# facebookresearch/theseus

Measured on NVIDIA H100. Metric: LM iterations/sec on batched SE3 pose-graph (2500 poses, global batch 2048 over N GPUs, LM + block-sparse Cholesky, fp64), higher is better.
Workload: dtype f64

## Files before the change

### include/thb200.h

```cpp
#ifndef THB200_H_
#define THB200_H_

#include <stdint.h>

#ifdef __cplusplus
extern "C" {
#endif

typedef struct CUstream_st* thb_stream_t;

#define THB_OK 0
#define THB_ERR_BAD_ARG (-1)
#define THB_ERR_UNSUPPORTED (-2)
#define THB_ERR_ALLOC (-3)

int thb_version(void);
int thb_compiled_arch(void);
int64_t thb_launch_count(void);

enum thb_cost_kind {
  THB_COST_BETWEEN_SE3 = 0,
  THB_COST_LOCAL_SE3 = 1,
  THB_COST_BETWEEN_SO3 = 2,
  THB_COST_LOCAL_SO3 = 3,
  THB_COST_LOCAL_VECTOR = 4,
  THB_COST_BETWEEN_SE2 = 6,
  THB_COST_LOCAL_SE2 = 7,
  THB_COST_REPROJECTION = 5
};
enum thb_robust_kind { THB_ROBUST_NONE = 0, THB_ROBUST_WELSCH = 1, THB_ROBUST_HUBER = 2 };
enum thb_weight_kind {
  THB_WEIGHT_SCALE = 0,
  THB_WEIGHT_DIAGONAL = 1
};
enum thb_var_kind { THB_VAR_SE3 = 0, THB_VAR_SO3 = 1, THB_VAR_VECTOR = 2, THB_VAR_SE2 = 3, THB_VAR_SO2 = 4 };

typedef struct thb_cost_group {
  int32_t kind;
  int32_t weight_kind;
  int32_t K;
  int32_t dim;
  const void* const* x0;
  const void* const* x1;
  const void* const* aux;
  const void* const* w;
  const int32_t* bstride;
  const int64_t* a_off;
  const int32_t* a_stride;
  const int32_t* bp;
  const int32_t* row0;
  const void* const* aux2;
  const void* const* aux3;
  const void* const* aux4;
  const int32_t* bstride2;
  int32_t robust_kind;
  int32_t reserved0;
  const void* const* log_radius;
  const int32_t* bstride_lr;
} thb_cost_group;

int thb_linearize_group_f64(const thb_cost_group* g, int64_t B, double* A_val, int64_t nnz, double* b, int64_t m,
                            thb_stream_t stream);
int thb_linearize_group_f32(const thb_cost_group* g, int64_t B, float* A_val, int64_t nnz, float* b, int64_t m,
                            thb_stream_t stream);

int thb_error_num_chunks(int32_t K);
int thb_error_group_f64(const thb_cost_group* g, int64_t B, double* partial, thb_stream_t stream);
int thb_error_group_f32(const thb_cost_group* g, int64_t B, float* partial, thb_stream_t stream);
int thb_error_reduce_f64(const double* partial, int32_t num_chunks, int64_t B, double* err, thb_stream_t stream);
int thb_error_reduce_f32(const float* partial, int32_t num_chunks, int64_t B, float* err, thb_stream_t stream);

typedef struct thb_var_table {
  int32_t N;
  const void* const* x;
  void* const* out;
  const int32_t* kind;
  const int32_t* col;
  const int32_t* dof;
} thb_var_table;

int thb_retract_f64(const thb_var_table* vt, int64_t B, const double* delta, int64_t n, double step,
                    const uint8_t* ignore , thb_stream_t stream);
int thb_retract_f32(const thb_var_table* vt, int64_t B, const float* delta, int64_t n, float step,
                    const uint8_t* ignore, thb_stream_t stream);
int thb_commit_f64(const thb_var_table* vt, int64_t B, const uint8_t* keep_old, thb_stream_t stream);
int thb_commit_f32(const thb_var_table* vt, int64_t B, const uint8_t* keep_old, thb_stream_t stream);

typedef struct thb_gram_plan {
  int64_t num_entries;
  const int32_t* ent_blk;
  const int16_t* ent_p;
  const int16_t* ent_q;
  const int64_t* blk_out;
  const int32_t* blk_ld;
  const int64_t* blk_mirror;
  const int32_t* blk_cptr;
  const int64_t* c_off;
  const int32_t* c_stride;
  const int32_t* c_rows;
  const int32_t* c_bpa;
  const int32_t* c_bpb;
  int64_t n;
  const int32_t* col_cptr;
  const int64_t* cc_off;
  const int32_t* cc_stride;
  const int32_t* cc_rows;
  const int32_t* cc_row0;
  int64_t num_blocks;
  const int32_t* blk_rows;
  const int32_t* blk_cols;
  int64_t num_segments;
  const int32_t* segments;
  const int32_t* blk_order;
} thb_gram_plan;

int thb_gram_f64(const thb_gram_plan* p, int64_t B, const double* A_val, int64_t nnz, const double* b, int64_t m,
                 double* out, int64_t out_bstride, double* Atb, double* diag, thb_stream_t stream);
int thb_gram_f32(const thb_gram_plan* p, int64_t B, const float* A_val, int64_t nnz, const float* b, int64_t m,
                 float* out, int64_t out_bstride, float* Atb, float* diag, thb_stream_t stream);
int thb_fill_zero(void* ptr, int64_t bytes, thb_stream_t stream);

int64_t thb_potrf_workspace_bytes(int64_t B, int64_t n);
int thb_potrf_f64(const double* AtA, const double* alpha, const double* beta, int32_t* info, int64_t B, int64_t n,
                  void* workspace, int64_t workspace_bytes, thb_stream_t stream);
int thb_potrs_f64(const double* rhs, double* x, int64_t B, int64_t n, const void* workspace, int64_t workspace_bytes,
                  thb_stream_t stream);
int thb_potrf_potrs_f64(const double* AtA, const double* rhs, const double* alpha, const double* beta, double* x,
                        int32_t* info, int64_t B, int64_t n, void* workspace, int64_t workspace_bytes,
                        thb_stream_t stream);

typedef struct thb_sparse_plan {
  int32_t N;
  int32_t num_levels;
  int32_t max_dim;
  int32_t reserved;
  int64_t n;
  int64_t data_size;
  int64_t winv_size;
  const int32_t* dims;
  const int32_t* col_start;
  const int32_t* pstart;
  const int64_t* winv_off;
  const int64_t* diag_off;
  const int64_t* up_a;
  const int64_t* up_b;
  const int32_t* up_k;
  const int64_t* u_ptr;
  const int64_t* u_tgt; const int16_t* u_r; const int16_t* u_c; const int16_t* u_ld; const int64_t* u_p0; const int64_t* u_p1;
  const int64_t* f_ptr;
  const int64_t* f_off; const int32_t* f_dim; const int64_t* f_w; const int32_t* f_col;
  const int64_t* t_ptr;
  const int64_t* t_off; const int16_t* t_r; const int16_t* t_dim; const int64_t* t_w;
  const int64_t* s_ptr;
  const int32_t* s_col;
  const int64_t* fr_ptr; const int64_t* fr_off; const int32_t* fr_k;
  const int64_t* bc_ptr; const int64_t* bc_off; const int32_t* bc_i;
} thb_sparse_plan;

int thb_sparse_damp_f64(const thb_sparse_plan* p, double* factor, const double* alpha, const double* beta, int64_t B,
                        thb_stream_t stream);
int thb_sparse_factor_f64(const thb_sparse_plan* p, double* factor, double* winv, int32_t* info, int64_t B, thb_stream_t stream);
int thb_sparse_solve_f64(const thb_sparse_plan* p, const double* factor, const double* winv, const double* rhs, double* x,
                         double* work, int64_t B, thb_stream_t stream);

typedef struct thb_symbolic thb_symbolic;
int thb_symbolic_create(const int64_t* param_size, int64_t N, const int64_t* blk_ptrs, const int64_t* blk_inds, int32_t ordering,
                        thb_symbolic** out);
void thb_symbolic_destroy(thb_symbolic* s);
int64_t thb_symbolic_array_count(const thb_symbolic* s, const char* name);
int32_t thb_symbolic_array_elem_bytes(const thb_symbolic* s, const char* name);
int thb_symbolic_array_copy(const thb_symbolic* s, const char* name, void* dst, int64_t dst_bytes);
double thb_symbolic_stat(const thb_symbolic* s, const char* name);

enum { THB_LANE_U = 0, THB_LANE_T = 1, THB_LANE_S = 2, THB_LANE_UH = 3, THB_LANE_TU = 4  };
typedef struct thb_sparse_lane_plan {
  int64_t N;
  int64_t n;
  int64_t data_size;
  int64_t diag_size;
  int64_t num_launches;
  const int32_t* launches;
  const int32_t* dims;
  const int32_t* col_start;
  const int32_t* pstart;
  const int64_t* dl_off;
  const int64_t* diag_off;
  const int64_t* up_a; const int64_t* up_b; const int32_t* up_k;
  const int64_t* u_tgt; const int64_t* u_p0; const int64_t* u_p1;
  const int64_t* t_off; const int64_t* t_diag; const int64_t* t_dl;
  const int32_t* t_pstart;
  const int32_t* s_col;
  const int64_t* fr_ptr; const int64_t* fr_off; const int32_t* fr_p; const int32_t* fr_d;
  const int64_t* bc_ptr; const int64_t* bc_off; const int32_t* bc_p; const int32_t* bc_d;
} thb_sparse_lane_plan;

int64_t thb_sparse_lane_padded_batch(int64_t B);
int thb_sparse_lane_gram_f64(const thb_gram_plan* g, int64_t B, const double* A_val, int64_t nnz, double* factor, thb_stream_t stream);
int thb_sparse_lane_damp_f64(const thb_sparse_lane_plan* p, double* factor, const double* alpha, const double* beta, int64_t B,
                             thb_stream_t stream);
int thb_sparse_lane_factor_f64(const thb_sparse_lane_plan* p, double* factor, double* diagl, int32_t* info, int64_t B,
                               thb_stream_t stream);
typedef struct thb_sparse_lane_root {
  int64_t num_blocks;
  int64_t num_cols;
  int64_t nt;
  int64_t root_start;
  int64_t num_segments;
  const int32_t* segments;
  const int64_t* rb_off; const int32_t* rb_row; const int32_t* rb_col; const int32_t* rb_di; const int32_t* rb_dj;
  const int64_t* rf_p0; const int64_t* rf_p1;
  const int32_t* root_cols;
  const int32_t* root_dims;
} thb_sparse_lane_root;
int thb_sparse_lane_root_gather_f64(const thb_sparse_lane_root* r, const double* factor, double* S, int64_t B, thb_stream_t stream);
int thb_sparse_lane_forward_f64(const thb_sparse_lane_plan* p, const double* factor, const double* diagl, const double* rhs, double* work,
                                int64_t B, thb_stream_t stream);
int thb_sparse_lane_backward_f64(const thb_sparse_lane_plan* p, const double* factor, const double* diagl, double* work, double* x, int64_t B,
                                 thb_stream_t stream);
int thb_sparse_lane_root_rhs_f64(const thb_sparse_lane_plan* p, const thb_sparse_lane_root* r, const double* factor, const double* rhs,
                                 const double* work, double* rhs_dense, int64_t B, thb_stream_t stream);
int thb_sparse_lane_root_scatter_f64(const thb_sparse_lane_plan* p, const thb_sparse_lane_root* r, const double* x_dense, double* work, double* x,
                                     int64_t B, thb_stream_t stream);
#define THB_TILE_ROWS 4
#define THB_TILE_COLS 4
typedef struct thb_sparse_lane_tiles {
  int64_t num_tiles, num_steps;
  const int64_t* tile_tgt;
  const int64_t* step_ptr;
  const int64_t* step_src;
} thb_sparse_lane_tiles;
int thb_sparse_lane_factor_tiled_f64(const thb_sparse_lane_plan* p, const thb_sparse_lane_tiles* t, double* factor, double* diagl,
                                     int32_t* info, int64_t B, thb_stream_t stream);
typedef struct thb_sparse_lane_pieces {
  int64_t num_pieces, num_launches;
  const int32_t* launches;
  const int64_t* first;
  const int32_t* width;
  const int64_t* fr_ext_end;
  const int64_t* bc_int_end;
  const int64_t* order;
} thb_sparse_lane_pieces;
int thb_sparse_lane_piece_forward_f64(const thb_sparse_lane_plan* p, const thb_sparse_lane_pieces* pc, const double* factor, const double* diagl,
                                      const double* rhs, double* work, int64_t B, thb_stream_t stream);
int thb_sparse_lane_piece_backward_f64(const thb_sparse_lane_plan* p, const thb_sparse_lane_pieces* pc, const double* factor, const double* diagl,
                                       double* work, double* x, int64_t B, thb_stream_t stream);
int thb_sparse_lane_solve_f64(const thb_sparse_lane_plan* p, const double* factor, const double* diagl, const double* rhs,
                              double* x, double* work, int64_t B, thb_stream_t stream);

int thb_lm_control_f64(const double* delta, const double* Atb, const double* diag, int64_t B, int64_t n, double step,
                       const double* err_prev, const double* err_new, double* lam, int32_t ellipsoidal,
                       double damping_accept, double down_ratio, double up_ratio, uint8_t* reject,
                       double* err_out, int32_t* stats, thb_stream_t stream);

int thb_lm_control_f32(const float* delta, const float* Atb, const float* diag, int64_t B, int64_t n, float step,
                       const float* err_prev, const float* err_new, float* lam, int32_t ellipsoidal, float damping_accept,
                       float down_ratio, float up_ratio, uint8_t* reject, float* err_out, int32_t* stats, thb_stream_t stream);

int thb_gram_dense_f64(const double* A, double* AtA, int64_t B, int64_t m, int64_t n, thb_stream_t stream);

typedef struct thb_front_plan {
  int64_t S;
  int64_t n;
  int64_t data_size;
  int64_t arena_size;
  int64_t varena_size;
  const int32_t* f_w; const int32_t* f_b; const int32_t* f_first; const int32_t* f_class;
  const int32_t* f_wpad; const int32_t* f_np; const int32_t* f_cb_ld; const int32_t* f_depth;
  const int64_t* f_panel_off; const int64_t* f_cb_off; const int64_t* f_fr_off; const int64_t* f_u_off;
  const int32_t* child_ptr; const int32_t* child_list;
  const int64_t* rel_ptr; const int32_t* f_rel;
  const int64_t* rows_ptr; const int32_t* f_rows;
  const int32_t* sched;
  const int32_t* perm;
  const int32_t* c_jw; const int64_t* c_sp_ptr; const int32_t* c_sp;
  const int64_t* c_inv_ptr; const int32_t* c_inv;
  const int64_t* fd; const int64_t* pc;
  const int32_t* pmap;
} thb_front_plan;

#define THB_FRONT_LAUNCH_COLS 12
int64_t thb_front_small_smem_bytes(int32_t w, int32_t b, int32_t nchildren);
int thb_front_factor_f64(const thb_front_plan* p, const int64_t* launches, int64_t num_launches, double* factor, const double* ata,
                         int64_t ata_stride, const double* alpha, const double* beta, double* arena, void* dense_ws, int64_t dense_ws_bytes,
                         int32_t* info, int64_t B, thb_stream_t stream);
int thb_front_solve_f64(const thb_front_plan* p, const int64_t* launches, int64_t num_launches, const double* factor, const double* rhs,
                        double* x, double* work, double* varena, int64_t B, thb_stream_t stream);
int64_t thb_potrf_partial_workspace_bytes(int64_t B, int64_t np);
int thb_potrf_partial_inplace_f64(double* F, int64_t bstride, int64_t np, int32_t nb_piv, int32_t w_real, int32_t n_real, int32_t info_base,
                                  int32_t* info, int64_t B, void* workspace, int64_t workspace_bytes, thb_stream_t stream);

int thb_mat_vec_f64(int64_t B, int64_t num_rows, int64_t num_cols, const int64_t* row_ptr, const int64_t* col_ind,
                    const double* A_val, const double* v, double* y, thb_stream_t stream);
int thb_tmat_vec_f64(int64_t B, int64_t num_rows, int64_t num_cols, const int64_t* row_ptr, const int64_t* col_ind,
                     const double* A_val, const double* v, double* y, thb_stream_t stream);

int thb_solve_backward_f64(int64_t B, int64_t num_rows, int64_t num_cols, const int64_t* row_ptr, const int64_t* col_ind,
                           const double* A_val, const double* b, const double* x, const double* H, const double* alpha,
                           int32_t detach_hessian, double* A_grad, double* b_grad, thb_stream_t stream);

int thb_se3_exp_f64(const double* tangent, double* group, int64_t N, thb_stream_t stream);
int thb_se3_log_f64(const double* group, double* tangent, double* jlog , int64_t N, thb_stream_t stream);
int thb_se3_adjoint_f64(const double* group, double* adj, int64_t N, thb_stream_t stream);
int thb_se3_inverse_f64(const double* group, double* out, int64_t N, thb_stream_t stream);
int thb_se3_compose_f64(const double* g0, const double* g1, double* out, int64_t N, thb_stream_t stream);
int thb_se3_exp_f32(const float* tangent, float* group, int64_t N, thb_stream_t stream);
int thb_se3_log_f32(const float* group, float* tangent, float* jlog, int64_t N, thb_stream_t stream);
int thb_se3_adjoint_f32(const float* group, float* adj, int64_t N, thb_stream_t stream);
int thb_se3_inverse_f32(const float* group, float* out, int64_t N, thb_stream_t stream);
int thb_se3_compose_f32(const float* g0, const float* g1, float* out, int64_t N, thb_stream_t stream);

int thb_so3_exp_f64(const double* tangent, double* group, int64_t N, thb_stream_t stream);
int thb_so3_log_f64(const double* group, double* tangent, double* jlog , int64_t N, thb_stream_t stream);
int thb_so3_adjoint_f64(const double* group, double* adj, int64_t N, thb_stream_t stream);
int thb_so3_inverse_f64(const double* group, double* out, int64_t N, thb_stream_t stream);
int thb_so3_compose_f64(const double* g0, const double* g1, double* out, int64_t N, thb_stream_t stream);
int thb_se2_exp_f64(const double* tangent, double* group, int64_t N, thb_stream_t stream);
int thb_se2_log_f64(const double* group, double* tangent, double* jlog , int64_t N, thb_stream_t stream);
int thb_se2_adjoint_f64(const double* group, double* adj, int64_t N, thb_stream_t stream);
int thb_se2_inverse_f64(const double* group, double* out, int64_t N, thb_stream_t stream);
int thb_se2_compose_f64(const double* g0, const double* g1, double* out, int64_t N, thb_stream_t stream);
int thb_so3_exp_f32(const float* tangent, float* group, int64_t N, thb_stream_t stream);
int thb_so3_log_f32(const float* group, float* tangent, float* jlog , int64_t N, thb_stream_t stream);
int thb_so3_adjoint_f32(const float* group, float* adj, int64_t N, thb_stream_t stream);
int thb_so3_inverse_f32(const float* group, float* out, int64_t N, thb_stream_t stream);
int thb_so3_compose_f32(const float* g0, const float* g1, float* out, int64_t N, thb_stream_t stream);
int thb_se2_exp_f32(const float* tangent, float* group, int64_t N, thb_stream_t stream);
int thb_se2_log_f32(const float* group, float* tangent, float* jlog , int64_t N, thb_stream_t stream);
int thb_se2_adjoint_f32(const float* group, float* adj, int64_t N, thb_stream_t stream);
int thb_se2_inverse_f32(const float* group, float* out, int64_t N, thb_stream_t stream);
int thb_se2_compose_f32(const float* g0, const float* g1, float* out, int64_t N, thb_stream_t stream);

int thb_so3_jexp_f64(const double* tangent, double* group , double* jexp, int64_t N, thb_stream_t stream);
int thb_se3_jexp_f64(const double* tangent, double* group , double* jexp, int64_t N, thb_stream_t stream);
int thb_so3_jexp_f32(const float* tangent, float* group , float* jexp, int64_t N, thb_stream_t stream);
int thb_se3_jexp_f32(const float* tangent, float* group , float* jexp, int64_t N, thb_stream_t stream);

#ifdef __cplusplus
}
#endif
#endif
```

### theseus_b200/_lib.py

```python
import ctypes as C
import os

_HERE = os.path.dirname(os.path.abspath(__file__))
_LIB_PATH = os.environ.get("THB200_LIB") or os.path.join(_HERE, "lib", "libthb200.so")
_lib = None

c_i32, c_i64, c_f64, c_f32, c_vp = C.c_int32, C.c_int64, C.c_double, C.c_float, C.c_void_p


class CostGroup(C.Structure):
    _fields_ = [("kind", c_i32), ("weight_kind", c_i32), ("K", c_i32), ("dim", c_i32),
                ("x0", c_vp), ("x1", c_vp), ("aux", c_vp), ("w", c_vp), ("bstride", c_vp),
                ("a_off", c_vp), ("a_stride", c_vp), ("bp", c_vp), ("row0", c_vp),
                ("aux2", c_vp), ("aux3", c_vp), ("aux4", c_vp), ("bstride2", c_vp),
                ("robust_kind", c_i32), ("reserved0", c_i32), ("log_radius", c_vp), ("bstride_lr", c_vp)]


class VarTable(C.Structure):
    _fields_ = [("N", c_i32), ("x", c_vp), ("out", c_vp), ("kind", c_vp), ("col", c_vp), ("dof", c_vp)]


class GramPlan(C.Structure):
    _fields_ = [("num_entries", c_i64), ("ent_blk", c_vp), ("ent_p", c_vp), ("ent_q", c_vp),
                ("blk_out", c_vp), ("blk_ld", c_vp), ("blk_mirror", c_vp), ("blk_cptr", c_vp),
                ("c_off", c_vp), ("c_stride", c_vp), ("c_rows", c_vp), ("c_bpa", c_vp), ("c_bpb", c_vp),
                ("n", c_i64), ("col_cptr", c_vp), ("cc_off", c_vp), ("cc_stride", c_vp), ("cc_rows", c_vp),
                ("cc_row0", c_vp), ("num_blocks", c_i64), ("blk_rows", c_vp), ("blk_cols", c_vp),
                ("num_segments", c_i64), ("segments", c_vp), ("blk_order", c_vp)]


def make_gram_plan(arrs, dev):
    return GramPlan(
        num_entries=int(arrs["ent_blk"].shape[0]), ent_blk=dev["ent_blk"].data_ptr(), ent_p=dev["ent_p"].data_ptr(),
        ent_q=dev["ent_q"].data_ptr(), blk_out=dev["blk_out"].data_ptr(), blk_ld=dev["blk_ld"].data_ptr(),
        blk_mirror=dev["blk_mirror"].data_ptr(), blk_cptr=dev["blk_cptr"].data_ptr(), c_off=dev["c_off"].data_ptr(),
        c_stride=dev["c_stride"].data_ptr(), c_rows=dev["c_rows"].data_ptr(), c_bpa=dev["c_bpa"].data_ptr(),
        c_bpb=dev["c_bpb"].data_ptr(), n=int(arrs["n"]), col_cptr=dev["col_cptr"].data_ptr(),
        cc_off=dev["cc_off"].data_ptr(), cc_stride=dev["cc_stride"].data_ptr(), cc_rows=dev["cc_rows"].data_ptr(),
        cc_row0=dev["cc_row0"].data_ptr(), num_blocks=int(arrs["blk_out"].shape[0]), blk_rows=dev["blk_rows"].data_ptr(),
        blk_cols=dev["blk_cols"].data_ptr(), num_segments=int(arrs["segments"].shape[0]), segments=arrs["segments"].ctypes.data,
        blk_order=dev["blk_order"].data_ptr())


class SparsePlanStruct(C.Structure):
    _fields_ = [("N", c_i32), ("num_levels", c_i32), ("max_dim", c_i32), ("reserved", c_i32),
                ("n", c_i64), ("data_size", c_i64), ("winv_size", c_i64)] + [(k, c_vp) for k in (
                    "dims", "col_start", "pstart", "winv_off", "diag_off", "up_a", "up_b", "up_k",
                    "u_ptr", "u_tgt", "u_r", "u_c", "u_ld", "u_p0", "u_p1",
                    "f_ptr", "f_off", "f_dim", "f_w", "f_col",
                    "t_ptr", "t_off", "t_r", "t_dim", "t_w",
                    "s_ptr", "s_col", "fr_ptr", "fr_off", "fr_k", "bc_ptr", "bc_off", "bc_i")]


class SparseLanePlanStruct(C.Structure):
    _fields_ = [("N", c_i64), ("n", c_i64), ("data_size", c_i64), ("diag_size", c_i64), ("num_launches", c_i64)] + [(k, c_vp) for k in (
        "launches", "dims", "col_start", "pstart", "dl_off", "diag_off", "up_a", "up_b", "up_k", "u_tgt", "u_p0", "u_p1",
        "t_off", "t_diag", "t_dl", "t_pstart", "s_col", "fr_ptr", "fr_off", "fr_p", "fr_d", "bc_ptr", "bc_off", "bc_p", "bc_d")]


_PG, _PV, _PP = C.POINTER(CostGroup), C.POINTER(VarTable), C.POINTER(GramPlan)
_PS = C.POINTER(SparsePlanStruct)
_PL = C.POINTER(SparseLanePlanStruct)


class SparseLaneRootStruct(C.Structure):
    _fields_ = [("num_blocks", c_i64), ("num_cols", c_i64), ("nt", c_i64), ("root_start", c_i64), ("num_segments", c_i64)] + [(k, c_vp) for k in (
        "segments", "rb_off", "rb_row", "rb_col", "rb_di", "rb_dj", "rf_p0", "rf_p1", "root_cols", "root_dims")]


class SparseLaneTilesStruct(C.Structure):
    _fields_ = [("num_tiles", c_i64), ("num_steps", c_i64), ("tile_tgt", c_vp), ("step_ptr", c_vp), ("step_src", c_vp)]


class SparseLanePiecesStruct(C.Structure):
    _fields_ = [("num_pieces", c_i64), ("num_launches", c_i64)] + [(k, c_vp) for k in (
        "launches", "first", "width", "fr_ext_end", "bc_int_end", "order")]


class FrontPlanStruct(C.Structure):
    _fields_ = [("S", c_i64), ("n", c_i64), ("data_size", c_i64), ("arena_size", c_i64), ("varena_size", c_i64)] + [(k, c_vp) for k in (
        "f_w", "f_b", "f_first", "f_class", "f_wpad", "f_np", "f_cb_ld", "f_depth", "f_panel_off", "f_cb_off", "f_fr_off", "f_u_off",
        "child_ptr", "child_list", "rel_ptr", "f_rel", "rows_ptr", "f_rows", "sched", "perm", "c_jw", "c_sp_ptr", "c_sp", "c_inv_ptr", "c_inv", "fd", "pc", "pmap")]


_PF = C.POINTER(FrontPlanStruct)
_PR = C.POINTER(SparseLaneRootStruct)
_PPIECES = C.POINTER(SparseLanePiecesStruct)
_PT = C.POINTER(SparseLaneTilesStruct)
SIGNATURES = {
    "thb_version": (c_i32, []),
    "thb_compiled_arch": (c_i32, []),
    "thb_launch_count": (c_i64, []),
    "thb_linearize_group_f64": (c_i32, [_PG, c_i64, c_vp, c_i64, c_vp, c_i64, c_vp]),
    "thb_linearize_group_f32": (c_i32, [_PG, c_i64, c_vp, c_i64, c_vp, c_i64, c_vp]),
    "thb_error_num_chunks": (c_i32, [c_i32]),
    "thb_error_group_f64": (c_i32, [_PG, c_i64, c_vp, c_vp]),
    "thb_error_group_f32": (c_i32, [_PG, c_i64, c_vp, c_vp]),
    "thb_error_reduce_f64": (c_i32, [c_vp, c_i32, c_i64, c_vp, c_vp]),
    "thb_error_reduce_f32": (c_i32, [c_vp, c_i32, c_i64, c_vp, c_vp]),
    "thb_retract_f64": (c_i32, [_PV, c_i64, c_vp, c_i64, c_f64, c_vp, c_vp]),
    "thb_retract_f32": (c_i32, [_PV, c_i64, c_vp, c_i64, c_f32, c_vp, c_vp]),
    "thb_commit_f64": (c_i32, [_PV, c_i64, c_vp, c_vp]),
    "thb_commit_f32": (c_i32, [_PV, c_i64, c_vp, c_vp]),
    "thb_gram_f64": (c_i32, [_PP, c_i64, c_vp, c_i64, c_vp, c_i64, c_vp, c_i64, c_vp, c_vp, c_vp]),
    "thb_gram_f32": (c_i32, [_PP, c_i64, c_vp, c_i64, c_vp, c_i64, c_vp, c_i64, c_vp, c_vp, c_vp]),
    "thb_fill_zero": (c_i32, [c_vp, c_i64, c_vp]),
    "thb_potrf_workspace_bytes": (c_i64, [c_i64, c_i64]),
    "thb_potrf_f64": (c_i32, [c_vp, c_vp, c_vp, c_vp, c_i64, c_i64, c_vp, c_i64, c_vp]),
    "thb_potrs_f64": (c_i32, [c_vp, c_vp, c_i64, c_i64, c_vp, c_i64, c_vp]),
    "thb_potrf_potrs_f64": (c_i32, [c_vp, c_vp, c_vp, c_vp, c_vp, c_vp, c_i64, c_i64, c_vp, c_i64, c_vp]),
    "thb_sparse_damp_f64": (c_i32, [_PS, c_vp, c_vp, c_vp, c_i64, c_vp]),
    "thb_sparse_factor_f64": (c_i32, [_PS, c_vp, c_vp, c_vp, c_i64, c_vp]),
    "thb_sparse_solve_f64": (c_i32, [_PS, c_vp, c_vp, c_vp, c_vp, c_vp, c_i64, c_vp]),
    "thb_symbolic_create": (c_i32, [c_vp, c_i64, c_vp, c_vp, c_i32, c_vp]),
    "thb_symbolic_destroy": (None, [c_vp]),
    "thb_symbolic_array_count": (c_i64, [c_vp, C.c_char_p]),
    "thb_symbolic_array_elem_bytes": (c_i32, [c_vp, C.c_char_p]),
    "thb_symbolic_array_copy": (c_i32, [c_vp, C.c_char_p, c_vp, c_i64]),
    "thb_symbolic_stat": (C.c_double, [c_vp, C.c_char_p]),
    "thb_sparse_lane_padded_batch": (c_i64, [c_i64]),
    "thb_sparse_lane_gram_f64": (c_i32, [_PP, c_i64, c_vp, c_i64, c_vp, c_vp]),
    "thb_sparse_lane_damp_f64": (c_i32, [_PL, c_vp, c_vp, c_vp, c_i64, c_vp]),
    "thb_sparse_lane_factor_f64": (c_i32, [_PL, c_vp, c_vp, c_vp, c_i64, c_vp]),
    "thb_sparse_lane_factor_tiled_f64": (c_i32, [_PL, _PT, c_vp, c_vp, c_vp, c_i64, c_vp]),
    "thb_sparse_lane_solve_f64": (c_i32, [_PL, c_vp, c_vp, c_vp, c_vp, c_vp, c_i64, c_vp]),
    "thb_sparse_lane_forward_f64": (c_i32, [_PL, c_vp, c_vp, c_vp, c_vp, c_i64, c_vp]),
    "thb_sparse_lane_backward_f64": (c_i32, [_PL, c_vp, c_vp, c_vp, c_vp, c_i64, c_vp]),
    "thb_sparse_lane_piece_forward_f64": (c_i32, [_PL, _PPIECES, c_vp, c_vp, c_vp, c_vp, c_i64, c_vp]),
    "thb_sparse_lane_piece_backward_f64": (c_i32, [_PL, _PPIECES, c_vp, c_vp, c_vp, c_vp, c_i64, c_vp]),
    "thb_sparse_lane_root_gather_f64": (c_i32, [_PR, c_vp, c_vp, c_i64, c_vp]),
    "thb_sparse_lane_root_rhs_f64": (c_i32, [_PL, _PR, c_vp, c_vp, c_vp, c_vp, c_i64, c_vp]),
    "thb_sparse_lane_root_scatter_f64": (c_i32, [_PL, _PR, c_vp, c_vp, c_vp, c_i64, c_vp]),
    "thb_gram_dense_f64": (c_i32, [c_vp, c_vp, c_i64, c_i64, c_i64, c_vp]),
    "thb_front_small_smem_bytes": (c_i64, [c_i32, c_i32, c_i32]),
    "thb_front_factor_f64": (c_i32, [_PF, c_vp, c_i64, c_vp, c_vp, c_i64, c_vp, c_vp, c_vp, c_vp, c_i64, c_vp, c_i64, c_vp]),
    "thb_front_solve_f64": (c_i32, [_PF, c_vp, c_i64, c_vp, c_vp, c_vp, c_vp, c_vp, c_i64, c_vp]),
    "thb_potrf_partial_workspace_bytes": (c_i64, [c_i64, c_i64]),
    "thb_potrf_partial_inplace_f64": (c_i32, [c_vp, c_i64, c_i64, c_i32, c_i32, c_i32, c_i32, c_vp, c_i64, c_vp, c_i64, c_vp]),
    "thb_solve_backward_f64": (c_i32, [c_i64, c_i64, c_i64, c_vp, c_vp, c_vp, c_vp, c_vp, c_vp, c_vp, c_i32, c_vp, c_vp, c_vp]),
    "thb_lm_control_f64": (c_i32, [c_vp, c_vp, c_vp, c_i64, c_i64, c_f64, c_vp, c_vp, c_vp, c_i32, c_f64, c_f64, c_f64,
                                   c_vp, c_vp, c_vp, c_vp]),
    "thb_lm_control_f32": (c_i32, [c_vp, c_vp, c_vp, c_i64, c_i64, c_f32, c_vp, c_vp, c_vp, c_i32, c_f32, c_f32, c_f32,
                                   c_vp, c_vp, c_vp, c_vp]),
    "thb_mat_vec_f64": (c_i32, [c_i64, c_i64, c_i64, c_vp, c_vp, c_vp, c_vp, c_vp, c_vp]),
    "thb_tmat_vec_f64": (c_i32, [c_i64, c_i64, c_i64, c_vp, c_vp, c_vp, c_vp, c_vp, c_vp]),
}
for _sfx, _ in (("f64", c_f64), ("f32", c_f32)):
    SIGNATURES[f"thb_se3_exp_{_sfx}"] = (c_i32, [c_vp, c_vp, c_i64, c_vp])
    SIGNATURES[f"thb_se3_log_{_sfx}"] = (c_i32, [c_vp, c_vp, c_vp, c_i64, c_vp])
    SIGNATURES[f"thb_se3_adjoint_{_sfx}"] = (c_i32, [c_vp, c_vp, c_i64, c_vp])
    SIGNATURES[f"thb_se3_inverse_{_sfx}"] = (c_i32, [c_vp, c_vp, c_i64, c_vp])
    SIGNATURES[f"thb_se3_compose_{_sfx}"] = (c_i32, [c_vp, c_vp, c_vp, c_i64, c_vp])
    SIGNATURES[f"thb_se3_jexp_{_sfx}"] = (c_i32, [c_vp, c_vp, c_vp, c_i64, c_vp])
    SIGNATURES[f"thb_so3_jexp_{_sfx}"] = (c_i32, [c_vp, c_vp, c_vp, c_i64, c_vp])
    for _g in ("so3", "se2"):
        SIGNATURES[f"thb_{_g}_exp_{_sfx}"] = (c_i32, [c_vp, c_vp, c_i64, c_vp])
        SIGNATURES[f"thb_{_g}_log_{_sfx}"] = (c_i32, [c_vp, c_vp, c_vp, c_i64, c_vp])
        SIGNATURES[f"thb_{_g}_adjoint_{_sfx}"] = (c_i32, [c_vp, c_vp, c_i64, c_vp])
        SIGNATURES[f"thb_{_g}_inverse_{_sfx}"] = (c_i32, [c_vp, c_vp, c_i64, c_vp])
        SIGNATURES[f"thb_{_g}_compose_{_sfx}"] = (c_i32, [c_vp, c_vp, c_vp, c_i64, c_vp])


def lib_path():
    return _LIB_PATH


def load():
    global _lib
    if _lib is not None:
        return _lib
    if not os.path.exists(_LIB_PATH):
        raise RuntimeError(
            f"libthb200.so not found at {_LIB_PATH}: build it with `python -m theseus_b200.build` "
            "(theseus_b200 has no CPU or PyTorch fallback for its compute path)")
    import torch
    lib = C.CDLL(_LIB_PATH, mode=C.RTLD_GLOBAL)
    for name, (res, args) in SIGNATURES.items():
        fn = getattr(lib, name)
        fn.restype = res
        fn.argtypes = args
    _lib = lib
    return lib


replayed_launches = 0


def total_launches() -> int:
    return int(load().thb_launch_count()) + replayed_launches


def check(rc, what):
    if rc != 0:
        kind = "invalid argument" if rc < 0 else "CUDA error"
        raise RuntimeError(f"libthb200: {what} failed with {kind} code {rc}")


def stream_ptr():
    import torch
    return C.c_void_p(torch.cuda.current_stream().cuda_stream)


def ptr(t):
    return None if t is None else C.c_void_p(t.data_ptr())
```

### theseus_b200/csrc/thb_front.cu

```cuda
#include <stdlib.h>

#include "thb_common.cuh"

namespace thb {

#ifdef THB_SIMT_EMU
#define THB_PDL_TRIGGER() do { } while (0)
#define THB_PDL_WAIT() do { } while (0)
#define FRONT_LAUNCH(K, grid, block, smem, cs, arg) K<<<grid, block, smem, cs>>>(arg)
#else
#define THB_PDL_TRIGGER() asm volatile("griddepcontrol.launch_dependents;" ::: "memory")
#define THB_PDL_WAIT() asm volatile("griddepcontrol.wait;" ::: "memory")
#define FRONT_LAUNCH(K, grid, block, smem, cs, arg) thb::front_launch_pdl(K, grid, block, smem, cs, arg)
static inline bool front_pdl_enabled() {
  static const bool on = [] { const char* e = getenv("THB_FRONT_PDL"); return e != nullptr && e[0] == '1'; }();
  return on;
}
template <typename A>
static inline void front_launch_pdl(void (*kernel)(A), dim3 grid, dim3 block, size_t smem, cudaStream_t cs, const A& arg) {
  cudaLaunchConfig_t cfg = {};
  cfg.gridDim = grid; cfg.blockDim = block; cfg.dynamicSmemBytes = smem; cfg.stream = cs;
  cudaLaunchAttribute at[1];
  at[0].id = cudaLaunchAttributeProgrammaticStreamSerialization;
  at[0].val.programmaticStreamSerializationAllowed = 1;
  cfg.attrs = at; cfg.numAttrs = front_pdl_enabled() ? 1 : 0;
  cudaLaunchKernelEx(&cfg, kernel, arg);
}
#endif

#ifdef THB_SIMT_EMU
__device__ inline void front_mma884(double& c0, double& c1, double a, double b) {
  const int lane = threadIdx.x & 31, lr = lane >> 2, lc = lane & 3;
  for (int k = 0; k < 4; k++) {
    const double av = __shfl_sync(0xffffffffu, a, lr * 4 + k);
    const double b0 = __shfl_sync(0xffffffffu, b, (2 * lc) * 4 + k);
    const double b1 = __shfl_sync(0xffffffffu, b, (2 * lc + 1) * 4 + k);
    c0 += av * b0;
    c1 += av * b1;
  }
}
#else
__device__ __forceinline__ void front_mma884(double& c0, double& c1, double a, double b) {
  asm volatile("mma.sync.aligned.m8n8k4.row.col.f64.f64.f64.f64 {%0,%1}, {%2}, {%3}, {%0,%1};\n" : "+d"(c0), "+d"(c1) : "d"(a), "d"(b));
}
#endif

__host__ __device__ __forceinline__ int front_pad_ld(int x) { return ((x + 11) / 16) * 16 + 4; }

struct FrontArgs {
  thb_front_plan p;
  int s0;
  int64_t B;
  double* factor;
  const double* alpha;
  const double* beta;
  double* arena_cur;
  const double* arena_child;
  int32_t* info;
  int prefetch;
  const double* ata;
  int64_t ata_stride;
};

__device__ __forceinline__ double front_panel_in(const FrontArgs& a, const double* Lg, int64_t poff, int64_t item, int64_t e) {
  if (a.ata == nullptr) return Lg[e];
  const int32_t m = a.p.pmap[poff + e];
  return m >= 0 ? a.ata[item * a.ata_stride + m] : 0.0;
}

constexpr int FRONT_WD_LD = 20;
#ifndef FRONT_PL
#define FRONT_PL 4
#endif
constexpr int FRONT_MAX_CHILDREN = 8;

__host__ __device__ __forceinline__ int64_t front_smem_doubles(int w, int b, int nchildren) {
  const int b16 = (b + 15) & ~15, w8 = (w + 7) & ~7;
  return (int64_t)(w8 + b16 + 8) * front_pad_ld(w8) + 8 * FRONT_WD_LD + 3 * FRONT_MAX_CHILDREN
         + ((int64_t)nchildren * (w + b) + 1) / 2 + 2;
}

__device__ __forceinline__ int front_leaf8(double* __restrict__ T, int ld, double* __restrict__ Wd, int lane) {
  const int ln = lane < 8 ? lane : 0;
  double row[8];
#pragma unroll
  for (int q = 0; q < 8; q++) row[q] = T[ln * ld + q];
  int fail = 0;
  double invd = 0.0;
#pragma unroll
  for (int c = 0; c < 8; c++) {
    const double d = __shfl_sync(0xffffffffu, row[c], c);
    if (!(d > 0.0) && fail == 0) fail = c + 1;
    double inv = rsqrt(d);
    inv = inv * (1.5 - 0.5 * d * inv * inv);
    const double sq = d * inv;
    if (lane == c) invd = inv;
    const double lrc = (lane == c) ? sq : row[c] * inv;
    row[c] = lrc;
#pragma unroll
    for (int q = c + 1; q < 8; q++) {
      const double lqc = __shfl_sync(0xffffffffu, lrc, q);
      row[q] -= lrc * lqc;
    }
  }
  if (lane < 8) {
#pragma unroll
    for (int q = 0; q < 8; q++)
      if (q <= lane) T[lane * ld + q] = row[q];
  }
  double x[8];
#pragma unroll
  for (int rr = 0; rr < 8; rr++) {
    double sacc = (lane == rr) ? 1.0 : 0.0;
#pragma unroll
    for (int k = 0; k < rr; k++) {
      const double lrk = __shfl_sync(0xffffffffu, row[k], rr);
      sacc -= lrk * x[k];
    }
    x[rr] = sacc * __shfl_sync(0xffffffffu, invd, rr);
  }
  if (lane < 8) {
#pragma unroll
    for (int rr = 0; rr < 8; rr++) Wd[rr * FRONT_WD_LD + lane] = (rr >= lane) ? x[rr] : 0.0;
  }
  return fail;
}

__device__ __forceinline__ void front_diag_block(double* PN, int ldp, int jb, double* Wd, int lane, int w, int first, int32_t* info) {
  const int lr = lane >> 2, lc = lane & 3;
  double c0 = 0.0, c1 = 0.0;
  const double* Arow = PN + (8 * jb + lr) * ldp + lc;
  for (int k = 0; k < 8 * jb; k += 4) {
    const double av = Arow[k];
    front_mma884(c0, c1, av, av);
  }
  double* d = PN + (8 * jb + lr) * ldp + 8 * jb + 2 * lc;
  d[0] -= c0;
  d[1] -= c1;
  __syncwarp();
  const int fail = front_leaf8(PN + (8 * jb) * ldp + 8 * jb, ldp, Wd, lane);
  if (lane == 0 && fail != 0 && 8 * jb + fail <= w) atomicCAS(info, 0, first + 8 * jb + fail);
}

template <bool TWO>
__device__ __forceinline__ void front_tile_column(double* PN, int ldp, int jb, int rt0, const double* Wd, int lane) {
  const int lr = lane >> 2, lc = lane & 3;
  double x00 = 0.0, x01 = 0.0, x10 = 0.0, x11 = 0.0;
  const double* A0 = PN + (8 * rt0 + lr) * ldp + lc;
  const double* Bj = PN + (8 * jb + lr) * ldp + lc;
  for (int k = 0; k < 8 * jb; k += 4) {
    const double bf = Bj[k];
    front_mma884(x00, x01, A0[k], bf);
    if (TWO) front_mma884(x10, x11, A0[8 * ldp + k], bf);
  }
  double* X0 = PN + (8 * rt0 + lr) * ldp + 8 * jb + 2 * lc;
  X0[0] -= x00; X0[1] -= x01;
  if (TWO) { X0[8 * ldp] -= x10; X0[8 * ldp + 1] -= x11; }
  __syncwarp();
  x00 = x01 = x10 = x11 = 0.0;
#pragma unroll
  for (int k = 0; k < 8; k += 4) {
    const double bf = Wd[lr * FRONT_WD_LD + k + lc];
    front_mma884(x00, x01, A0[8 * jb + k], bf);
    if (TWO) front_mma884(x10, x11, A0[8 * ldp + 8 * jb + k], bf);
  }
  __syncwarp();
  X0[0] = x00; X0[1] = x01;
  if (TWO) { X0[8 * ldp] = x10; X0[8 * ldp + 1] = x11; }
}

struct FrontChild {
  const double* src;
  int ldg, lo, hi, pad;
};

template <int THREADS>
__global__ void __launch_bounds__(THREADS, 1024 / THREADS) front_small_kernel(FrontArgs a) {
  extern __shared__ double sm[];
  const thb_front_plan& p = a.p;
  const int tid = threadIdx.x, lane = tid & 31, warp = tid >> 5;
  constexpr int NW = THREADS / 32;
  const int lr = lane >> 2, lc = lane & 3;
  const int64_t item = blockIdx.x;
  THB_PDL_TRIGGER();
  const int64_t* FD = p.fd + (int64_t)(a.s0 + blockIdx.y) * 8;
  const int t = (int)FD[0];
  const int w = (int)FD[1], b = (int)FD[2], r = w + b;
  const int f_first = (int)FD[3];
  const int64_t f_panel_off = FD[4], f_cb_off = FD[5];
  const int f_cb_ld = (int)FD[6];
  const int c_begin = (int)(FD[7] & 0xffffffffLL);
  const int nch = min((int)(FD[7] >> 32), FRONT_MAX_CHILDREN);
  (void)t;
  const int b16 = (b + 15) & ~15, w8 = (w + 7) & ~7;
  const int ldp = front_pad_ld(w8);
  const int prow = w8 + b16 + 8;
  double* PN = sm;
  double* Wd = PN + prow * ldp;
  FrontChild* ch = reinterpret_cast<FrontChild*>(Wd + 8 * FRONT_WD_LD);
  int32_t* INV = reinterpret_cast<int32_t*>(Wd + 8 * FRONT_WD_LD + 3 * FRONT_MAX_CHILDREN);
  for (int q = 0; q < nch; q++) {
    const int64_t* PC = p.pc + (int64_t)(c_begin + q) * 6;
    const double* csrc = a.arena_child + item * p.arena_size + PC[0];
    const int cld = (int)(PC[1] & 0xffffffffLL), cbc = (int)(PC[1] >> 32);
    if (tid == 0) {
      ch[q].src = csrc;
      ch[q].ldg = cld;
      ch[q].lo = (int)PC[2];
      ch[q].hi = (int)PC[3];
    }
    const int32_t* inv = p.c_inv + PC[4];
    for (int l = tid; l < r; l += THREADS) INV[q * r + l] = inv[l];
    (void)cbc;
  }
  for (int e = tid; e < prow * ldp; e += THREADS) sm[e] = 0.0;
  THB_PDL_WAIT();
#ifndef THB_SIMT_EMU
  for (int q = 0; a.prefetch != 0 && q < nch; q++) {
    const int64_t* PC = p.pc + (int64_t)(c_begin + q) * 6;
    const double* csrc = a.arena_child + item * p.arena_size + PC[0];
    const int cld = (int)(PC[1] & 0xffffffffLL), cbc = (int)(PC[1] >> 32);
    for (int off = tid * 16; off < cbc * cld; off += THREADS * 16) {
      const int i = off / cld, j = off - i * cld;
      if (j <= i) asm volatile("prefetch.global.L2 [%0];\n" ::"l"(csrc + off));
    }
  }
#endif
  __syncthreads();
  if (tid < w8 - w) PN[(w + tid) * ldp + w + tid] = 1.0;
  double* Lg = a.factor + item * p.data_size + f_panel_off;
  {
    const double al = a.alpha != nullptr ? a.alpha[item] : 0.0;
    const double be = a.beta != nullptr ? a.beta[item] : 0.0;
    const int total = r * w;
    for (int e0 = tid; e0 < total; e0 += FRONT_PL * THREADS) {
      int ii[FRONT_PL], jj[FRONT_PL];
      double v[FRONT_PL];
#pragma unroll
      for (int u = 0; u < FRONT_PL; u++) {
        const int e = e0 + u * THREADS;
        ii[u] = e / w;
        jj[u] = e - ii[u] * w;
        if (e >= total || jj[u] > ii[u]) ii[u] = -1;
        v[u] = ii[u] >= 0 ? front_panel_in(a, Lg, f_panel_off, item, e) : 0.0;
      }
#pragma unroll
      for (int u = 0; u < FRONT_PL; u++)
        if (ii[u] >= 0 && ii[u] == jj[u]) v[u] = v[u] + (al * v[u] + be);
      for (int q = 0; q < nch; q++) {
        const double* src = ch[q].src;
        const int ldg = ch[q].ldg, lo = ch[q].lo, hi = ch[q].hi;
        const int32_t* inv = INV + q * r;
#pragma unroll
        for (int u = 0; u < FRONT_PL; u++) {
          if (ii[u] >= lo && jj[u] <= hi) {
            const int ci = inv[ii[u]], cj = inv[jj[u]];
            if (ci >= 0 && cj >= 0) v[u] += src[(int64_t)ci * ldg + cj];
          }
        }
      }
#pragma unroll
      for (int u = 0; u < FRONT_PL; u++)
        if (ii[u] >= 0) PN[(ii[u] < w ? ii[u] : ii[u] + (w8 - w)) * ldp + jj[u]] = v[u];
    }
  }
  __syncthreads();
  const int nbk = w8 / 8, nrt = (w8 + b16) / 8;
  for (int jb = 0; jb < nbk; jb++) {
    if (warp == 0) front_diag_block(PN, ldp, jb, Wd, lane, w, f_first, a.info + item);
    __syncthreads();
    const int npair = (nrt - jb) / 2;
    for (int q = warp; q < npair; q += NW) front_tile_column<true>(PN, ldp, jb, jb + 1 + 2 * q, Wd, lane);
    __syncthreads();
  }
  {
    int i = tid / w, j = tid - i * w;
    const int di = THREADS / w, dj = THREADS - di * w;
    for (int e = tid; e < r * w; e += THREADS) {
      Lg[e] = (j > i) ? 0.0 : PN[(i < w ? i : i + (w8 - w)) * ldp + j];
      i += di; j += dj;
      if (j >= w) { j -= w; i++; }
    }
  }
  if (b == 0) return;
  double* dst = a.arena_cur + item * p.arena_size + f_cb_off;
  const int ldg_out = f_cb_ld;
  const double* P = PN + w8 * ldp;
  const int nmt = b16 / 16, ntl = nmt * (nmt + 1) / 2;
  for (int q = warp; q < ntl; q += NW) {
    int R = (int)((sqrtf(8.0f * (float)q + 1.0f) - 1.0f) * 0.5f);
    while ((R + 1) * (R + 2) / 2 <= q) R++;
    while (R * (R + 1) / 2 > q) R--;
    const int ct = q - R * (R + 1) / 2;
    double gch[2][2][2] = {{{0.0, 0.0}, {0.0, 0.0}}, {{0.0, 0.0}, {0.0, 0.0}}};
    const int li0 = w + 16 * R + lr, lj0 = w + 16 * ct + 2 * lc;
    for (int qc = 0; qc < nch; qc++) {
      if (w + 16 * R + 15 >= ch[qc].lo && w + 16 * ct <= ch[qc].hi) {
        const int32_t* inv = INV + qc * r;
        const double* src = ch[qc].src;
        const int ldg = ch[qc].ldg;
        int ci[2], cj[2][2];
#pragma unroll
        for (int mi = 0; mi < 2; mi++) ci[mi] = (li0 + 8 * mi < r) ? inv[li0 + 8 * mi] : -1;
#pragma unroll
        for (int ni = 0; ni < 2; ni++)
#pragma unroll
          for (int u = 0; u < 2; u++) cj[ni][u] = (lj0 + 8 * ni + u < r) ? inv[lj0 + 8 * ni + u] : -1;
#pragma unroll
        for (int mi = 0; mi < 2; mi++)
#pragma unroll
          for (int ni = 0; ni < 2; ni++)
#pragma unroll
            for (int u = 0; u < 2; u++)
              if (ci[mi] >= 0 && cj[ni][u] >= 0 && cj[ni][u] <= ci[mi]) gch[mi][ni][u] += src[(int64_t)ci[mi] * ldg + cj[ni][u]];
      }
    }
    double acc[2][2][2] = {{{0.0, 0.0}, {0.0, 0.0}}, {{0.0, 0.0}, {0.0, 0.0}}};
    const double* Pa = P + (16 * R + lr) * ldp + lc;
    const double* Pb = P + (16 * ct + lr) * ldp + lc;
    for (int k4 = 0; k4 < w8; k4 += 4) {
      const double a0 = Pa[k4], a1 = Pa[8 * ldp + k4];
      const double b0 = Pb[k4], b1 = Pb[8 * ldp + k4];
      front_mma884(acc[0][0][0], acc[0][0][1], a0, b0);
      front_mma884(acc[0][1][0], acc[0][1][1], a0, b1);
      front_mma884(acc[1][0][0], acc[1][0][1], a1, b0);
      front_mma884(acc[1][1][0], acc[1][1][1], a1, b1);
    }
#pragma unroll
    for (int mi = 0; mi < 2; mi++)
#pragma unroll
      for (int ni = 0; ni < 2; ni++) {
        acc[mi][ni][0] = gch[mi][ni][0] - acc[mi][ni][0];
        acc[mi][ni][1] = gch[mi][ni][1] - acc[mi][ni][1];
      }
#pragma unroll
    for (int mi = 0; mi < 2; mi++) {
      const int i = 16 * R + 8 * mi + lr;
      if (i < b) {
        double* drow = dst + (int64_t)i * ldg_out;
#pragma unroll
        for (int ni = 0; ni < 2; ni++)
#pragma unroll
          for (int u = 0; u < 2; u++) {
            const int jj = 16 * ct + 8 * ni + 2 * lc + u;
            if (jj <= i) drow[jj] = acc[mi][ni][u];
          }
      }
    }
  }
}

constexpr int ASM_ROWS = 16, ASM_THREADS = 256;

__device__ __forceinline__ int front_map_big(int l, int w, int wpad) { return l < w ? l : wpad + (l - w); }

__global__ void __launch_bounds__(ASM_THREADS) front_assemble_kernel(FrontArgs a, int t) {
  extern __shared__ double sm[];
  const thb_front_plan& p = a.p;
  const int tid = threadIdx.x;
  const int64_t item = blockIdx.x;
  const int w = p.f_w[t], b = p.f_b[t], r = w + b, wpad = p.f_wpad[t], np = p.f_np[t];
  const int R0 = blockIdx.y * ASM_ROWS;
  const int nc = min(np, 128 * (R0 / 128 + 1));
  const int c_first = p.child_ptr[t], n_children = p.child_ptr[t + 1] - c_first;
  if (n_children <= FRONT_MAX_CHILDREN) {
    const double* Lgg = a.factor + item * p.data_size + p.f_panel_off[t];
    const double alg = a.alpha != nullptr ? a.alpha[item] : 0.0;
    const double beg = a.beta != nullptr ? a.beta[item] : 0.0;
    double* Fg = a.arena_cur + item * p.arena_size + p.f_fr_off[t] + (int64_t)R0 * np;
    __shared__ const double* s_src[FRONT_MAX_CHILDREN];
    __shared__ const int32_t* s_inv[FRONT_MAX_CHILDREN];
    __shared__ int s_ld[FRONT_MAX_CHILDREN];
    if (tid < n_children) {
      const int c = p.child_list[c_first + tid];
      s_src[tid] = a.arena_child + item * p.arena_size + p.f_cb_off[c];
      s_inv[tid] = p.c_inv + p.c_inv_ptr[c];
      s_ld[tid] = p.f_cb_ld[c];
    }
    __syncthreads();
    const int64_t poff = p.f_panel_off[t];
    const int total = ASM_ROWS * nc;
    for (int e0 = tid; e0 < total; e0 += 4 * ASM_THREADS) {
      int li[4], lj[4];
      double v[4];
#pragma unroll
      for (int u = 0; u < 4; u++) {
        const int e = e0 + u * ASM_THREADS;
        const int rr = e / nc, fc = e - rr * nc;
        const int fr = R0 + rr;
        li[u] = fr < w ? fr : ((fr >= wpad && fr - wpad + w < r) ? fr - wpad + w : -1);
        lj[u] = fc < w ? fc : ((fc >= wpad && fc - wpad + w < r) ? fc - wpad + w : -1);
        v[u] = 0.0;
        if (e >= total) {
          li[u] = lj[u] = -2;
        } else if (li[u] < 0 || lj[u] < 0) {
          v[u] = (fr == fc) ? 1.0 : 0.0;
          li[u] = -1;
        } else if (lj[u] > li[u]) {
          li[u] = -1;
        } else if (lj[u] < w) {
          v[u] = front_panel_in(a, Lgg, poff, item, (int64_t)li[u] * w + lj[u]);
        }
      }
#pragma unroll
      for (int u = 0; u < 4; u++)
        if (li[u] >= 0 && li[u] == lj[u] && lj[u] < w) v[u] = v[u] + (alg * v[u] + beg);
      for (int q = 0; q < n_children; q++) {
        const double* src = s_src[q];
        const int32_t* inv = s_inv[q];
        const int ldg = s_ld[q];
        int ci[4], cj[4];
#pragma unroll
        for (int u = 0; u < 4; u++) {
          ci[u] = li[u] >= 0 ? inv[li[u]] : -1;
          cj[u] = li[u] >= 0 ? inv[lj[u]] : -1;
        }
#pragma unroll
        for (int u = 0; u < 4; u++)
          if (ci[u] >= 0 && cj[u] >= 0) v[u] += src[(int64_t)ci[u] * ldg + cj[u]];
      }
#pragma unroll
      for (int u = 0; u < 4; u++) {
        const int e = e0 + u * ASM_THREADS;
        if (e < total) Fg[e + (int64_t)(e / nc) * (np - nc)] = v[u];
      }
    }
    return;
  }
  double* buf = sm;
  for (int e = tid; e < ASM_ROWS * nc; e += ASM_THREADS) buf[e] = 0.0;
  __syncthreads();
  const double* Lg = a.factor + item * p.data_size + p.f_panel_off[t];
  const double al = a.alpha != nullptr ? a.alpha[item] : 0.0;
  const double be = a.beta != nullptr ? a.beta[item] : 0.0;
  const int wlim = min(wpad, nc);
  for (int e = tid; e < ASM_ROWS * wlim; e += ASM_THREADS) {
    const int rr = e / wlim, j = e - rr * wlim;
    const int fr = R0 + rr;
    int i = -1;
    if (fr < w) i = fr;
    else if (fr >= wpad && fr - wpad + w < r) i = fr - wpad + w;
    if (i >= 0) {
      if (j < w && !(i < w && j > i)) {
        double v = front_panel_in(a, Lg, p.f_panel_off[t], item, (int64_t)i * w + j);
        if (i == j) v = v + (al * v + be);
        buf[rr * nc + j] = v;
      }
    } else if (j == fr) {
      buf[rr * nc + j] = 1.0;
    }
  }
  for (int rr = tid; rr < ASM_ROWS; rr += ASM_THREADS) {
    const int fr = R0 + rr;
    if (fr >= wpad + b) buf[rr * nc + fr] = 1.0;
  }
  __syncthreads();
  for (int ci = p.child_ptr[t]; ci < p.child_ptr[t + 1]; ci++) {
    const int c = p.child_list[ci];
    const int bc = p.f_b[c], ldg = p.f_cb_ld[c];
    const int32_t* rel = p.f_rel + p.rel_ptr[c];
    int lo = 0, hi = bc;
    while (lo < hi) { const int mid = (lo + hi) >> 1; if (front_map_big(rel[mid], w, wpad) < R0) lo = mid + 1; else hi = mid; }
    const int i0 = lo;
    hi = bc;
    while (lo < hi) { const int mid = (lo + hi) >> 1; if (front_map_big(rel[mid], w, wpad) < R0 + ASM_ROWS) lo = mid + 1; else hi = mid; }
    const int i1 = lo;
    if (i1 > i0) {
      const double* src = a.arena_child + item * p.arena_size + p.f_cb_off[c];
      for (int i = i0 + (tid >> 5); i < i1; i += ASM_THREADS / 32) {
        const int fr = front_map_big(rel[i], w, wpad) - R0;
        const double* srow = src + (int64_t)i * ldg;
        for (int j = tid & 31; j <= i; j += 32) buf[fr * nc + front_map_big(rel[j], w, wpad)] += srow[j];
      }
      __syncthreads();
    }
  }
  double* F = a.arena_cur + item * p.arena_size + p.f_fr_off[t] + (int64_t)R0 * np;
  for (int e = tid; e < ASM_ROWS * nc; e += ASM_THREADS) {
    const int rr = e / nc, c = e - rr * nc;
    F[(int64_t)rr * np + c] = buf[e];
  }
}

__global__ void __launch_bounds__(256) front_extract_kernel(FrontArgs a, int t) {
  const thb_front_plan& p = a.p;
  const int64_t item = blockIdx.x;
  const int w = p.f_w[t], b = p.f_b[t], r = w + b, wpad = p.f_wpad[t], np = p.f_np[t];
  const double* F = a.arena_cur + item * p.arena_size + p.f_fr_off[t];
  double* Lg = a.factor + item * p.data_size + p.f_panel_off[t];
  for (int e = blockIdx.y * blockDim.x + threadIdx.x; e < r * w; e += gridDim.y * blockDim.x) {
    const int i = e / w, j = e - i * w;
    const int fr = i < w ? i : wpad + (i - w);
    Lg[e] = (i < w && j > i) ? 0.0 : F[(int64_t)fr * np + j];
  }
}

struct FrontSolveArgs {
  thb_front_plan p;
  int s0;
  int64_t B;
  const double* factor;
  const double* rhs;
  double* x;
  double* work;
  double* v_cur;
  const double* v_child;
  int stage_doubles;
};

__device__ __forceinline__ double front_warp_trsv_lower(const double* T, double ui, int cw, int lane) {
  const double rd = lane < cw ? 1.0 / T[lane * 33 + lane] : 0.0;
  for (int k = 0; k < cw; k++) {
    const double yk = __shfl_sync(0xffffffffu, ui * rd, k);
    if (lane == k) ui = yk;
    else if (lane > k && lane < cw) ui -= T[lane * 33 + k] * yk;
  }
  return ui;
}
__device__ __forceinline__ double front_warp_trsv_upper(const double* T, double ti, int cw, int lane) {
  const double rd = lane < cw ? 1.0 / T[lane * 33 + lane] : 0.0;
  for (int k = cw - 1; k >= 0; k--) {
    const double xk = __shfl_sync(0xffffffffu, ti * rd, k);
    if (lane == k) ti = xk;
    else if (lane < k) ti -= T[k * 33 + lane] * xk;
  }
  return ti;
}

template <int THREADS>
__global__ void __launch_bounds__(THREADS) front_forward_kernel(FrontSolveArgs a) {
  extern __shared__ double sm[];
  const thb_front_plan& p = a.p;
  const int tid = threadIdx.x, lane = tid & 31, warp = tid >> 5;
  const int64_t item = blockIdx.x;
  THB_PDL_TRIGGER();
  const int64_t* FD = p.fd + (int64_t)(a.s0 + blockIdx.y) * 8;
  const int t = (int)FD[0];
  const int w = (int)FD[1], b = (int)FD[2], r = w + b, first = (int)FD[3];
  THB_PDL_WAIT();
  double* u = sm;
  double* T = sm + ((r + 1) & ~1);
  const double* Lg = a.factor + item * p.data_size + FD[4];
  if (r * w <= a.stage_doubles) {
    double* Ls = T + 32 * 33 + 1 + (THREADS & ~1) + 2;
    for (int e = tid; e < r * w; e += THREADS) Ls[e] = Lg[e];
    Lg = Ls;
  }
  {
    const int c0 = (int)(FD[7] & 0xffffffffLL), nchild = (int)(FD[7] >> 32);
    for (int i = tid; i < r; i += THREADS) {
      double v = i < w ? a.rhs[item * p.n + p.perm[first + i]] : 0.0;
      for (int q = 0; q < nchild; q++) {
        const int64_t* PC = p.pc + (int64_t)(c0 + q) * 6;
        if (i >= (int)PC[2] && i <= (int)PC[3]) {
          const int k = p.c_inv[PC[4] + i];
          if (k >= 0) v += a.v_child[item * p.varena_size + PC[5] + k];
        }
      }
      u[i] = v;
    }
  }
  __syncthreads();
  for (int k0 = 0; k0 < w; k0 += 32) {
    const int cw = min(32, w - k0);
    for (int e = tid; e < cw * cw; e += THREADS) {
      const int i = e / cw, j = e - i * cw;
      T[i * 33 + j] = Lg[(int64_t)(k0 + i) * w + k0 + j];
    }
    __syncthreads();
    if (warp == 0) {
      const double ui = front_warp_trsv_lower(T, lane < cw ? u[k0 + lane] : 0.0, cw, lane);
      if (lane < cw) u[k0 + lane] = ui;
    }
    __syncthreads();
    for (int i = k0 + cw + tid; i < r; i += THREADS) {
      const double* row = Lg + (int64_t)i * w + k0;
      double s = 0.0;
      for (int k = 0; k < cw; k++) s += row[k] * u[k0 + k];
      u[i] -= s;
    }
    __syncthreads();
  }
  for (int i = tid; i < w; i += THREADS) a.work[item * p.n + first + i] = u[i];
  if (b > 0) {
    double* ub = a.v_cur + item * p.varena_size + p.f_u_off[t];
    for (int i = tid; i < b; i += THREADS) ub[i] = u[w + i];
  }
}

template <int THREADS>
__global__ void __launch_bounds__(THREADS) front_backward_kernel(FrontSolveArgs a) {
  extern __shared__ double sm[];
  const thb_front_plan& p = a.p;
  const int tid = threadIdx.x, lane = tid & 31, warp = tid >> 5;
  const int64_t item = blockIdx.x;
  THB_PDL_TRIGGER();
  const int64_t* FD = p.fd + (int64_t)(a.s0 + blockIdx.y) * 8;
  const int t = (int)FD[0];
  const int w = (int)FD[1], b = (int)FD[2], r = w + b, first = (int)FD[3];
  THB_PDL_WAIT();
  double* xf = sm;
  double* T = sm + ((r + 1) & ~1);
  double* part = T + 32 * 33 + 1;
  const double* Lg = a.factor + item * p.data_size + FD[4];
  if (r * w <= a.stage_doubles) {
    double* Ls = T + 32 * 33 + 1 + (THREADS & ~1) + 2;
    for (int e = tid; e < r * w; e += THREADS) Ls[e] = Lg[e];
    Lg = Ls;
  }
  double* wk = a.work + item * p.n;
  const int32_t* rows = p.f_rows + p.rows_ptr[t];
  for (int i = tid; i < r; i += THREADS) xf[i] = i < w ? wk[first + i] : wk[rows[i - w]];
  __syncthreads();
  const int nchunk = (w + 31) / 32;
  for (int ch = nchunk - 1; ch >= 0; ch--) {
    const int k0 = ch * 32, cw = min(32, w - k0);
    const int RG = THREADS / cw;
    const int kk = tid % cw, rg = tid / cw;
    for (int e = tid; e < cw * cw; e += THREADS) {
      const int i = e / cw, j = e - i * cw;
      T[i * 33 + j] = Lg[(int64_t)(k0 + i) * w + k0 + j];
    }
    double acc = 0.0;
    if (rg < RG) {
      const double* col = Lg + k0 + kk;
      int i = k0 + cw + rg;
      for (; i + 3 * RG < r; i += 4 * RG) {
        const double l0 = col[(int64_t)i * w], l1 = col[(int64_t)(i + RG) * w], l2 = col[(int64_t)(i + 2 * RG) * w],
                     l3 = col[(int64_t)(i + 3 * RG) * w];
        acc += l0 * xf[i];
        acc += l1 * xf[i + RG];
        acc += l2 * xf[i + 2 * RG];
        acc += l3 * xf[i + 3 * RG];
      }
      for (; i < r; i += RG) acc += col[(int64_t)i * w] * xf[i];
    }
    part[tid] = acc;
    __syncthreads();
    if (warp == 0) {
      double tk = 0.0;
      if (lane < cw) {
        tk = xf[k0 + lane];
        for (int g = 0; g < RG; g++) tk -= part[g * cw + lane];
      }
      tk = front_warp_trsv_upper(T, tk, cw, lane);
      if (lane < cw) xf[k0 + lane] = tk;
    }
    __syncthreads();
  }
  for (int i = tid; i < w; i += THREADS) {
    const double v = xf[i];
    wk[first + i] = v;
    a.x[item * p.n + p.perm[first + i]] = v;
  }
}

static inline int front_threads_of_class(int cls) { return cls == 0 ? 64 : (cls == 1 ? 128 : 256); }

template <typename K>
static inline int front_set_smem(K kernel, size_t bytes, size_t* cache) {
  if (bytes > *cache) {
    cudaError_t e = cudaFuncSetAttribute(kernel, cudaFuncAttributeMaxDynamicSharedMemorySize, (int)bytes);
    if (e != cudaSuccess) return (int)e;
    *cache = bytes;
  }
  return 0;
}

}

extern "C" {

int64_t thb_front_small_smem_bytes(int32_t w, int32_t b, int32_t nchildren) { return thb::front_smem_doubles(w, b, nchildren) * 8; }

int thb_front_factor_f64(const thb_front_plan* p, const int64_t* launches, int64_t num_launches, double* factor, const double* ata,
                         int64_t ata_stride, const double* alpha, const double* beta, double* arena, void* dense_ws, int64_t dense_ws_bytes,
                         int32_t* info, int64_t B, thb_stream_t stream) {
  if (p == nullptr || launches == nullptr || factor == nullptr || arena == nullptr || info == nullptr || B < 0) return THB_ERR_BAD_ARG;
  if (B == 0 || p->S == 0) return THB_OK;
  if (B > 65535LL * 32768LL) return THB_ERR_UNSUPPORTED;
  cudaStream_t cs = thb_cs(stream);
  THB_CUDA(cudaMemsetAsync(info, 0, (size_t)B * 4, cs));
  static size_t smem_set[5] = {0, 0, 0, 0, 0}, asm_set = 0;
  static const int thr_cls[2] = {[] { const char* e = getenv("THB_FRONT_T0"); const int v = e ? atoi(e) : 64; return (v == 128 || v == 256) ? v : 64; }(),
                                 [] { const char* e = getenv("THB_FRONT_T1"); const int v = e ? atoi(e) : 128; return v == 256 ? 256 : 128; }()};
  static int front_prefetch_flag = -1;
  if (front_prefetch_flag < 0) {
    const char* e = getenv("THB_FRONT_PREFETCH");
    front_prefetch_flag = (e != nullptr && e[0] == '0') ? 0 : 1;
  }
  for (int64_t l = 0; l < num_launches; l++) {
    const int64_t* L = launches + l * THB_FRONT_LAUNCH_COLS;
    const int depth = (int)L[0], cls = (int)L[1], begin = (int)L[2], count = (int)L[3];
    thb::FrontArgs a;
    a.p = *p; a.s0 = begin; a.B = B; a.factor = factor; a.alpha = alpha; a.beta = beta; a.info = info;
    a.ata = (ata != nullptr && p->pmap != nullptr) ? ata : nullptr; a.ata_stride = ata_stride;
    a.prefetch = front_prefetch_flag;
    a.arena_cur = arena + (int64_t)(depth & 1) * B * p->arena_size;
    a.arena_child = arena + (int64_t)((depth + 1) & 1) * B * p->arena_size;
    if (cls < 3) {
      const size_t smem = (size_t)L[4];
#ifndef THB_SIMT_EMU
      if (smem > 227 * 1024) return THB_ERR_UNSUPPORTED;
#endif
      const dim3 grid((unsigned)B, (unsigned)count);
      if (count > 65535) return THB_ERR_UNSUPPORTED;
      if (cls == 0 && thr_cls[0] == 64) {
        int rc = thb::front_set_smem(thb::front_small_kernel<64>, smem, &smem_set[0]); if (rc) return rc;
        FRONT_LAUNCH(thb::front_small_kernel<64>, grid, 64, smem, cs, a);
      } else if ((cls == 0 && thr_cls[0] == 128) || (cls == 1 && thr_cls[1] == 128)) {
        int rc = thb::front_set_smem(thb::front_small_kernel<128>, smem, &smem_set[1]); if (rc) return rc;
        FRONT_LAUNCH(thb::front_small_kernel<128>, grid, 128, smem, cs, a);
      } else if (cls <= 1 || smem <= 56 * 1024) {
        int rc = thb::front_set_smem(thb::front_small_kernel<256>, smem, &smem_set[2]); if (rc) return rc;
        FRONT_LAUNCH(thb::front_small_kernel<256>, grid, 256, smem, cs, a);
      } else if (smem <= 113 * 1024) {
        int rc = thb::front_set_smem(thb::front_small_kernel<512>, smem, &smem_set[3]); if (rc) return rc;
        FRONT_LAUNCH(thb::front_small_kernel<512>, grid, 512, smem, cs, a);
      } else {
        int rc = thb::front_set_smem(thb::front_small_kernel<1024>, smem, &smem_set[4]); if (rc) return rc;
        FRONT_LAUNCH(thb::front_small_kernel<1024>, grid, 1024, smem, cs, a);
      }
      THB_CHECK_LAUNCH();
    } else {
      const int64_t np = L[5], nb_piv = L[6], fr_off = L[7], first = L[8];
      const int t = (int)L[9];
#ifdef THB_SIMT_EMU
      (void)np; (void)nb_piv; (void)fr_off; (void)first; (void)t; (void)dense_ws; (void)dense_ws_bytes; (void)asm_set;
      return THB_ERR_UNSUPPORTED;
#else
      if (dense_ws == nullptr || np % 128 != 0 || np > 8192) return THB_ERR_BAD_ARG;
      const size_t smem = (size_t)thb::ASM_ROWS * np * 8;
      int rc = thb::front_set_smem(thb::front_assemble_kernel, smem, &asm_set); if (rc) return rc;
      thb::front_assemble_kernel<<<dim3((unsigned)B, (unsigned)(np / thb::ASM_ROWS)), thb::ASM_THREADS, smem, cs>>>(a, t);
      THB_CHECK_LAUNCH();
      rc = thb_potrf_partial_inplace_f64(a.arena_cur + fr_off, p->arena_size, np, (int32_t)nb_piv, (int32_t)L[10], (int32_t)(nb_piv * 64 + L[11]),
                                         (int32_t)first, info, B, dense_ws, dense_ws_bytes, stream);
      if (rc != THB_OK) return rc;
      thb::front_extract_kernel<<<dim3((unsigned)B, 8), 256, 0, cs>>>(a, t);
      THB_CHECK_LAUNCH();
#endif
    }
  }
  return THB_OK;
}

int thb_front_solve_f64(const thb_front_plan* p, const int64_t* launches, int64_t num_launches, const double* factor, const double* rhs,
                        double* x, double* work, double* varena, int64_t B, thb_stream_t stream) {
  if (p == nullptr || launches == nullptr || factor == nullptr || rhs == nullptr || x == nullptr || work == nullptr || varena == nullptr ||
      B < 0)
    return THB_ERR_BAD_ARG;
  if (B == 0 || p->S == 0) return THB_OK;
  cudaStream_t cs = thb_cs(stream);
  static size_t fw_set[3] = {0, 0, 0}, bw_set[3] = {0, 0, 0};
  static const int64_t stage_cap = [] { const char* e = getenv("THB_SOLVE_STAGE"); return e != nullptr ? (int64_t)atoll(e) : (int64_t)0; }();
  for (int pass = 0; pass < 2; pass++) {
    for (int64_t q = 0; q < num_launches; q++) {
      const int64_t l = pass == 0 ? q : num_launches - 1 - q;
      const int64_t* L = launches + l * THB_FRONT_LAUNCH_COLS;
      const int depth = (int)L[0], cls = (int)L[1], begin = (int)L[2], count = (int)L[3];
      thb::FrontSolveArgs a;
      a.p = *p; a.s0 = begin; a.B = B; a.factor = factor; a.rhs = rhs; a.x = x; a.work = work;
      a.v_cur = varena + (int64_t)(depth & 1) * B * p->varena_size;
      a.v_child = varena + (int64_t)((depth + 1) & 1) * B * p->varena_size;
      const int kc = cls > 2 ? 2 : cls;
      const int threads = thb::front_threads_of_class(kc);
      const int64_t r_max = L[5];
      const int64_t stage = (cls < 3 && L[6] > 0) ? (L[6] < stage_cap ? L[6] : stage_cap) : 0;
      a.stage_doubles = (int)stage;
      const size_t smem = (size_t)(((r_max + 1) & ~1LL) + 32 * 33 + 1 + threads + 2 + stage + 2) * 8;
      const dim3 grid((unsigned)B, (unsigned)count);
      if (pass == 0) {
        if (kc == 0) { int rc = thb::front_set_smem(thb::front_forward_kernel<64>, smem, &fw_set[0]); if (rc) return rc;
                       FRONT_LAUNCH(thb::front_forward_kernel<64>, grid, 64, smem, cs, a); }
        else if (kc == 1) { int rc = thb::front_set_smem(thb::front_forward_kernel<128>, smem, &fw_set[1]); if (rc) return rc;
                            FRONT_LAUNCH(thb::front_forward_kernel<128>, grid, 128, smem, cs, a); }
        else { int rc = thb::front_set_smem(thb::front_forward_kernel<256>, smem, &fw_set[2]); if (rc) return rc;
               FRONT_LAUNCH(thb::front_forward_kernel<256>, grid, 256, smem, cs, a); }
      } else {
        if (kc == 0) { int rc = thb::front_set_smem(thb::front_backward_kernel<64>, smem, &bw_set[0]); if (rc) return rc;
                       FRONT_LAUNCH(thb::front_backward_kernel<64>, grid, 64, smem, cs, a); }
        else if (kc == 1) { int rc = thb::front_set_smem(thb::front_backward_kernel<128>, smem, &bw_set[1]); if (rc) return rc;
                            FRONT_LAUNCH(thb::front_backward_kernel<128>, grid, 128, smem, cs, a); }
        else { int rc = thb::front_set_smem(thb::front_backward_kernel<256>, smem, &bw_set[2]); if (rc) return rc;
               FRONT_LAUNCH(thb::front_backward_kernel<256>, grid, 256, smem, cs, a); }
      }
      THB_CHECK_LAUNCH();
    }
  }
  return THB_OK;
}

}
```

### theseus_b200/sparse_solver.py

```python
import ctypes as C
import os
from typing import Any, Dict, Optional, Type, Union

import numpy as np
import torch

from . import _lib
from .autograd import LinearSolveFunction, wants_grad
from .core import Objective
from .optimizer import (Linearization, LinearSolver, SparseLinearization, convert_to_alpha_beta_damping_tensors)
from .frontal import build_front_plan
from .sparse import LANE_DIMS, analyze, gram_out_offsets, piece_solve_lists, root_lane_lists, root_split, tile_lane_lists
from .structure import ata_block_structure, build_gram_plan


_ROOT_LAYOUTS = ("lane_root", "lane_tiled_root")
_TILED_LAYOUTS = ("lane_tiled", "lane_tiled_root")


class BaspachoSparseSolver(LinearSolver):
    def __init__(self, objective: Objective, linearization_cls: Optional[Type[Linearization]] = None,
                 linearization_kwargs: Optional[Dict[str, Any]] = None, num_solver_contexts=1, batch_size: Optional[int] = None,
                 auto_reset: bool = True, dev: Optional[str] = None, ordering: str = "mindeg", layout: Optional[str] = None,
                 supernodal_solve: bool = False, front_options: Optional[Dict[str, Any]] = None, **kwargs):
        linearization_cls = linearization_cls or SparseLinearization
        if not linearization_cls == SparseLinearization:
            raise RuntimeError(
                "BaspachoSparseSolver only works with theseus.optimizer.SparseLinearization,"
                + f" got {type(self.linearization)}")
        super().__init__(objective, linearization_cls, linearization_kwargs, **kwargs)
        self.linearization: SparseLinearization = self.linearization
        self._ordering = ordering
        self._layout = layout
        self._supernodal_solve = bool(supernodal_solve)
        self._front_options = dict(front_options or {})
        self._plan = None
        self._dev = None
        self.param_size = None
        self.reset()

    @classmethod
    def from_structure(cls, structure, ordering: str = "mindeg", layout: Optional[str] = None,
                       supernodal_solve: bool = False, front_options: Optional[Dict[str, Any]] = None) -> "BaspachoSparseSolver":
        class _Lin:
            def __init__(self, S):
                self._S, self.A_val, self.b = S, None, None
                self.A_row_ptr, self.A_col_ind = S.A_row_ptr, S.A_col_ind
                self.num_rows, self.num_cols = S.num_rows, S.num_cols

            def structure(self):
                return self._S
        self = cls.__new__(cls)
        self.linearization = _Lin(structure)
        self._ordering, self._plan, self._dev, self._layout = ordering, None, None, layout
        self._supernodal_solve = bool(supernodal_solve)
        self._front_options = dict(front_options or {})
        self.param_size = None
        self.reset()
        return self

    def reset(self, **kwargs):
        if self._plan is not None:
            return
        S = self.linearization.structure()
        if getattr(self, "param_size", None) is None:
            param_size, ptrs, inds = ata_block_structure(S)
            self.param_size, self.block_ptrs, self.block_inds = param_size, ptrs, inds
        param_size, ptrs, inds = self.param_size, self.block_ptrs, self.block_inds
        if self._layout is None:
            return
        if self._layout == "front":
            opts = {k: v for k, v in getattr(self, "_front_options", {}).items() if k != "chunk"}
            for env, key, cast in (("THB_FRONT_TAU", "tau", float), ("THB_FRONT_MERGE_FLOPS", "merge_flops", float),
                                   ("THB_FRONT_MERGE_MAX_R", "merge_max_r", int)):
                if env in os.environ and key not in opts:
                    opts[key] = cast(os.environ[env])
            self._plan = build_front_plan(param_size, ptrs, inds, ordering="auto" if self._ordering == "mindeg" else self._ordering, **opts)
            from .structure import lower_blocks
            blocks, _ = lower_blocks(S, self._plan.pos)
            dims_of = S.var_dims
            f, self._ata_size = self._plan.gram_compact_offsets([(a, b, int(dims_of[a]), int(dims_of[b])) for a, b in blocks])
            self._gram_arrays = build_gram_plan(S, out_offsets=f, pos=self._plan.pos)
            return
        self._plan = analyze(param_size, ptrs, inds, ordering=self._ordering)
        self._gram_arrays = build_gram_plan(S, out_offsets=gram_out_offsets(self._plan), pos=self._plan.pos)

    def layout_for(self, B: int) -> str:
        if self._layout is None:
            self._layout = os.environ.get("THB_SPARSE_LAYOUT") or ("front" if B >= 32 else "item")
            self.reset()
        if self._layout == "front":
            return "front"
        lane_ok = all(int(d) in LANE_DIMS for d in self._plan.dims)
        if self._layout is not None:
            if self._layout not in ("lane", "item", "lane_root", "lane_tiled", "lane_tiled_root"):
                raise ValueError(f"layout must be 'lane', 'item', 'lane_root', 'lane_tiled' or 'lane_tiled_root', got {self._layout}")
            if self._layout != "item" and not lane_ok:
                raise ValueError(f"layout='{self._layout}' needs block sizes in {LANE_DIMS}")
            if self._layout in _ROOT_LAYOUTS and self._root_split() is None:
                raise ValueError(f"layout='{self._layout}': this structure has no dense root (top chain too short)")
            return self._layout
        return "lane" if (lane_ok and B >= 32) else "item"

    def _root_split(self):
        if not hasattr(self, "_root"):
            sp = root_split(self._plan)
            self._root = None if sp is None else (sp,) + root_lane_lists(self._plan, sp)
        return self._root

    @property
    def symbolic_stats(self):
        if self._plan is None:
            self._layout = os.environ.get("THB_SPARSE_LAYOUT") or "front"
            self.reset()
        return dict(self._plan.stats)

    @property
    def effective_layout(self):
        return self._layout

    def _device_plan(self, device):
        if self._dev is not None and self._dev["device"] == device:
            return self._dev
        if self._layout == "front":
            return self._device_plan_front(device)
        P = self._plan
        dev = {k: torch.from_numpy(np.ascontiguousarray(v)).to(device) for k, v in P.arrays.items()}
        st = _lib.SparsePlanStruct(N=P.N, num_levels=int(P.stats["levels"]), max_dim=int(P.dims.max()) if P.N else 0, reserved=0,
                                   n=P.n, data_size=P.data_size, winv_size=P.winv_size,
                                   **{k: dev[k].data_ptr() for k in dev})
        g = self._gram_arrays
        gdev = {k: torch.from_numpy(np.ascontiguousarray(v)).to(device) for k, v in g.items() if isinstance(v, np.ndarray)}
        gst = _lib.make_gram_plan(g, gdev)
        ln = P.lane
        lst, ldev, launches = self._lane_struct(ln, dev, device)
        self._dev = dict(device=device, plan=st, keep=dev, gram=gst, gkeep=gdev, bufs={}, lane=lst, lkeep=(ldev, launches))
        if self._layout in _ROOT_LAYOUTS:
            sp, rl, rr = self._root_split()
            qdev = {k: torch.from_numpy(np.ascontiguousarray(v)).to(device) for k, v in rr.items() if isinstance(v, np.ndarray) and k != "segments"}
            segs = np.ascontiguousarray(rr["segments"], dtype=np.int32)
            qst = _lib.SparseLaneRootStruct(
                num_blocks=int(rr["rb_off"].shape[0]), num_cols=int(rr["root_cols"].shape[0]), nt=int(rr["nt"]), root_start=int(rr["root_start"]),
                num_segments=int(segs.shape[0]), segments=segs.ctypes.data, rb_off=qdev["rb_off"].data_ptr(), rb_row=qdev["rb_row"].data_ptr(),
                rb_col=qdev["rb_col"].data_ptr(), rb_di=qdev["rb_di"].data_ptr(), rb_dj=qdev["rb_dj"].data_ptr(), rf_p0=qdev["rf_p0"].data_ptr(),
                rf_p1=qdev["rf_p1"].data_ptr(), root_cols=qdev["root_cols"].data_ptr(), root_dims=qdev["root_dims"].data_ptr())
            self._dev.update(root=qst, qkeep=(qdev, segs), nt=int(rr["nt"]))
            if self._layout == "lane_root":
                rst, rdev, rlaunch = self._lane_struct(rl, dev, device)
                self._dev.update(lane_root=rst, rkeep=(rdev, rlaunch))
        if self._layout in _TILED_LAYOUTS:
            tl, tt = self._tile_lists()
            tst, tdev, tlaunch = self._lane_struct(tl, dev, device)
            ttdev = {k: torch.from_numpy(np.ascontiguousarray(v)).to(device) for k, v in tt.items()}
            tiles = _lib.SparseLaneTilesStruct(num_tiles=int(tt["tile_tgt"].shape[0]), num_steps=int(tt["step_src"].shape[0]),
                                               tile_tgt=ttdev["tile_tgt"].data_ptr(), step_ptr=ttdev["step_ptr"].data_ptr(),
                                               step_src=ttdev["step_src"].data_ptr())
            self._dev.update({self._layout: tst}, tiles=tiles, tkeep=(tdev, tlaunch, ttdev))
        if getattr(self, "_supernodal_solve", False) and all(int(d) in LANE_DIMS for d in P.dims):
            ps = piece_solve_lists(P, cut=self._root_split()[0]["cut"] if self._layout in _ROOT_LAYOUTS else None)
            pdev = {k: torch.from_numpy(np.ascontiguousarray(ps[k] if k != "width" else ps[k].astype(np.int32))).to(device)
                    for k in ("first", "width", "fr_ext_end", "bc_int_end", "order")}
            plaunch = np.ascontiguousarray(ps["launches"][:, 1:], dtype=np.int32)
            pst = _lib.SparseLanePiecesStruct(num_pieces=int(ps["first"].shape[0]), num_launches=int(plaunch.shape[0]), launches=plaunch.ctypes.data,
                                              **{k: pdev[k].data_ptr() for k in pdev})
            self._dev.update(pieces=pst, pkeep=(pdev, plaunch, ps))
        return self._dev

    def _device_plan_front(self, device):
        P = self._plan
        dev = {k: torch.from_numpy(np.ascontiguousarray(v)).to(device) for k, v in P.arrays.items()}
        st = _lib.FrontPlanStruct(S=P.S, n=P.n, data_size=P.data_size, arena_size=P.arena_size, varena_size=P.varena_size,
                                  **{k: dev[k].data_ptr() for k in ("f_w", "f_b", "f_first", "f_class", "f_wpad", "f_np", "f_cb_ld", "f_depth",
                                                                    "f_panel_off", "f_cb_off", "f_fr_off", "f_u_off", "child_ptr", "child_list",
                                                                    "rel_ptr", "f_rel", "rows_ptr", "f_rows", "sched", "perm", "c_jw", "c_sp_ptr", "c_sp", "c_inv_ptr", "c_inv", "fd", "pc", "pmap")})
        g = self._gram_arrays
        gdev = {k: torch.from_numpy(np.ascontiguousarray(v)).to(device) for k, v in g.items() if isinstance(v, np.ndarray)}
        launches = np.ascontiguousarray(P.launches, dtype=np.int64)
        big = launches[launches[:, 1] == 3]
        self._dev = dict(device=device, front=st, keep=dev, gram=_lib.make_gram_plan(g, gdev), gkeep=gdev, bufs={}, launches=launches,
                         max_np=int(big[:, 5].max()) if len(big) else 0)
        return self._dev

    def _numeric_front(self, A_val, b, alpha, beta):
        B, device = A_val.shape[0], A_val.device
        d = self._device_plan(device)
        P = self._plan
        lib = _lib.load()
        s = _lib.stream_ptr()
        chunk = int(min(B, self._front_options.get("chunk", int(os.environ.get("THB_FRONT_CHUNK", "1024")))))
        if d["bufs"].get("key") != (B, "front"):
            ws_bytes = int(lib.thb_potrf_partial_workspace_bytes(chunk, d["max_np"])) if d["max_np"] else 0
            d["bufs"] = dict(key=(B, "front"), chunk=chunk, factor=torch.empty(B, P.data_size, dtype=torch.float64, device=device),
                             ata=torch.empty(B, self._ata_size, dtype=torch.float64, device=device),
                             arena=torch.empty(2, chunk, P.arena_size, dtype=torch.float64, device=device),
                             varena=torch.empty(2, chunk, P.varena_size, dtype=torch.float64, device=device),
                             work=torch.empty(B, P.n, dtype=torch.float64, device=device),
                             ws=torch.empty(max(ws_bytes, 8), dtype=torch.uint8, device=device),
                             Atb=torch.empty(B, P.n, dtype=torch.float64, device=device),
                             AtA_diag=torch.empty(B, P.n, dtype=torch.float64, device=device),
                             info=torch.empty(B, dtype=torch.int32, device=device))
        bufs = d["bufs"]
        factor, Atb, info = bufs["factor"], bufs["Atb"], bufs["info"]
        lin = self.linearization
        if getattr(lin, "_Atb", None) is Atb:
            lin._Atb = lin._AtA_diag = None
        nnz, m = A_val.shape[1], b.shape[1]
        self._factor_stamp = getattr(self, "_factor_stamp", 0) + 1
        ata = bufs["ata"]
        _lib.check(lib.thb_gram_f64(C.byref(d["gram"]), B, _lib.ptr(A_val), nnz, _lib.ptr(b), m, _lib.ptr(ata), self._ata_size,
                                    _lib.ptr(Atb), _lib.ptr(bufs["AtA_diag"]), s), "gram(front)")
        L = d["launches"]
        for c0 in range(0, B, chunk):
            nb = min(chunk, B - c0)
            _lib.check(lib.thb_front_factor_f64(
                C.byref(d["front"]), L.ctypes.data, L.shape[0], _lib.ptr(factor[c0:]), _lib.ptr(ata[c0:]), self._ata_size,
                _lib.ptr(alpha[c0:]) if alpha is not None else None,
                _lib.ptr(beta[c0:]) if beta is not None else None, _lib.ptr(bufs["arena"]), _lib.ptr(bufs["ws"]) if d["max_np"] else None,
                bufs["ws"].numel(), _lib.ptr(info[c0:]), nb, s), "front_factor")
        self._keep = (A_val, b, alpha, beta)
        return Atb

    def _substitute_front(self, rhs):
        d, P = self._dev, self._plan
        bufs = d["bufs"]
        B, chunk = bufs["key"][0], bufs["chunk"]
        lib = _lib.load()
        rhs = rhs.contiguous()
        x = torch.empty(B, P.n, dtype=torch.float64, device=rhs.device)
        L = d["launches"]
        for c0 in range(0, B, chunk):
            nb = min(chunk, B - c0)
            _lib.check(lib.thb_front_solve_f64(C.byref(d["front"]), L.ctypes.data, L.shape[0], _lib.ptr(bufs["factor"][c0:]), _lib.ptr(rhs[c0:]),
                                               _lib.ptr(x[c0:]), _lib.ptr(bufs["work"][c0:]), _lib.ptr(bufs["varena"]), nb, _lib.stream_ptr()),
                       "front_solve")
        return x

    def _lane_struct(self, ln, dev, device):
        P = self._plan
        ldev = {k: torch.from_numpy(np.ascontiguousarray(v)).to(device) for k, v in ln.items() if k != "launches"}
        launches = np.ascontiguousarray(ln["launches"], dtype=np.int32)
        lst = _lib.SparseLanePlanStruct(
            N=P.N, n=P.n, data_size=P.data_size, diag_size=P.winv_size, num_launches=int(launches.shape[0]),
            launches=launches.ctypes.data, dims=dev["dims"].data_ptr(), col_start=dev["col_start"].data_ptr(),
            pstart=dev["pstart"].data_ptr(), dl_off=dev["winv_off"].data_ptr(), diag_off=dev["diag_off"].data_ptr(),
            up_a=dev["up_a"].data_ptr(), up_b=dev["up_b"].data_ptr(), up_k=dev["up_k"].data_ptr(),
            u_tgt=ldev["u_tgt"].data_ptr(), u_p0=ldev["u_p0"].data_ptr(), u_p1=ldev["u_p1"].data_ptr(),
            t_off=ldev["t_off"].data_ptr(), t_diag=ldev["t_diag"].data_ptr(), t_dl=ldev["t_dl"].data_ptr(),
            t_pstart=ldev["t_pstart"].data_ptr(), s_col=ldev["s_col"].data_ptr(),
            fr_ptr=dev["fr_ptr"].data_ptr(), fr_off=dev["fr_off"].data_ptr(), fr_p=ldev["fr_p"].data_ptr(), fr_d=ldev["fr_d"].data_ptr(),
            bc_ptr=dev["bc_ptr"].data_ptr(), bc_off=dev["bc_off"].data_ptr(), bc_p=ldev["bc_p"].data_ptr(), bc_d=ldev["bc_d"].data_ptr())
        return lst, ldev, launches

    def _tile_lists(self):
        if not hasattr(self, "_tiles"):
            self._tiles = tile_lane_lists(self._plan, self._root_split()[0] if self._layout in _ROOT_LAYOUTS else None)
        return self._tiles

    def solve(self, damping: Optional[Union[float, torch.Tensor]] = None, ellipsoidal_damping: bool = True,
              damping_eps: float = 1e-8, **kwargs) -> torch.Tensor:
        lin = self.linearization
        A_val, b = lin.A_val, lin.b
        if A_val is None:
            raise RuntimeError("linearize() must be called before solve()")
        if wants_grad(A_val, b):
            detach = bool(getattr(lin, "detached_hessian", False))
            return LinearSolveFunction.apply(A_val, b, self, damping, ellipsoidal_damping, damping_eps, detach)
        x = self._solve_nograd(A_val, b, damping, ellipsoidal_damping, damping_eps)[0]
        bufs = self._dev["bufs"] if self._dev is not None else {}
        if "AtA_diag" in bufs and A_val.dtype == torch.float64 and A_val.is_contiguous() and b.is_contiguous() and getattr(lin, "_Atb", 0) is None:
            lin._Atb, lin._AtA_diag = bufs["Atb"], bufs["AtA_diag"]
        return x

    def _solve_nograd(self, A_val, b, damping, ellipsoidal_damping, damping_eps):
        out_dtype = A_val.dtype
        A64, b64 = A_val.detach(), b.detach()
        if A64.dtype != torch.float64:
            A64, b64 = A64.double(), b64.double()
        A64, b64 = A64.contiguous(), b64.contiguous()
        alpha = beta = None
        if damping is not None:
            alpha, beta = convert_to_alpha_beta_damping_tensors(damping, damping_eps, ellipsoidal_damping, A64.shape[0], A64.device, torch.float64)
        Atb = self._numeric(A64, b64, alpha, beta)
        x = self._substitute(Atb)
        self._last_info = self._dev["bufs"]["info"]
        if not getattr(self, "defer_info_check", False):
            self.check_info()
        return x.to(out_dtype), (A64, b64, x, alpha, beta)

    def check_info(self, x=None):
        self._raise_if_bad(self._last_info)
        return x

    @staticmethod
    def _raise_if_bad(info):
        bad = info.nonzero()
        if bad.numel() > 0:
            k = int(bad[0, 0])
            raise RuntimeError(f"block-sparse Cholesky: batch element {k}: matrix is not positive definite (pivot {int(info[k])})")

    def _numeric(self, A_val, b, alpha, beta):
        B, device = A_val.shape[0], A_val.device
        layout = self.layout_for(B)
        if layout == "front":
            return self._numeric_front(A_val, b, alpha, beta)
        d = self._device_plan(device)
        P = self._plan
        lib = _lib.load()
        s = _lib.stream_ptr()
        key = (B, layout)
        if d["bufs"].get("key") != key:
            Bp = int(lib.thb_sparse_lane_padded_batch(B))
            shape = (lambda k: (k, Bp)) if layout != "item" else (lambda k: (B, k))
            d["bufs"] = dict(key=key, factor=torch.empty(shape(P.data_size), dtype=torch.float64, device=device),
                             diag=torch.empty(shape(P.winv_size), dtype=torch.float64, device=device),
                             work=torch.empty(shape(P.n), dtype=torch.float64, device=device),
                             Atb=torch.empty(B, P.n, dtype=torch.float64, device=device),
                             info=torch.empty(B, dtype=torch.int32, device=device))
            if layout in _ROOT_LAYOUTS:
                nt = d["nt"]
                d["bufs"].update(S=torch.empty(B, nt, nt, dtype=torch.float64, device=device),
                                 ws=torch.empty(int(lib.thb_potrf_workspace_bytes(B, nt)), dtype=torch.uint8, device=device),
                                 rhs_root=torch.empty(B, nt, dtype=torch.float64, device=device),
                                 x_root=torch.empty(B, nt, dtype=torch.float64, device=device),
                                 info_root=torch.empty(B, dtype=torch.int32, device=device))
        bufs = d["bufs"]
        factor, diag, Atb, info = bufs["factor"], bufs["diag"], bufs["Atb"], bufs["info"]
        nnz, m = A_val.shape[1], b.shape[1]
        self._factor_stamp = getattr(self, "_factor_stamp", 0) + 1
        _lib.check(lib.thb_fill_zero(_lib.ptr(factor), factor.numel() * 8, s), "fill_zero")
        if layout != "item":
            lplan = d[layout]
            _lib.check(lib.thb_sparse_lane_gram_f64(C.byref(d["gram"]), B, _lib.ptr(A_val), nnz, _lib.ptr(factor), s), "gram(lane)")
            _lib.check(lib.thb_gram_f64(C.byref(d["gram"]), B, _lib.ptr(A_val), nnz, _lib.ptr(b), m, None, 0, _lib.ptr(Atb), None, s), "Atb")
            if alpha is not None:
                _lib.check(lib.thb_sparse_lane_damp_f64(C.byref(d["lane"]), _lib.ptr(factor), _lib.ptr(alpha), _lib.ptr(beta), B, s), "lane_damp")
            if layout in _TILED_LAYOUTS:
                _lib.check(lib.thb_sparse_lane_factor_tiled_f64(C.byref(lplan), C.byref(d["tiles"]), _lib.ptr(factor), _lib.ptr(diag), _lib.ptr(info),
                                                                B, s), "lane_factor_tiled")
            else:
                _lib.check(lib.thb_sparse_lane_factor_f64(C.byref(lplan), _lib.ptr(factor), _lib.ptr(diag), _lib.ptr(info), B, s), "lane_factor")
            if layout in _ROOT_LAYOUTS:
                _lib.check(lib.thb_sparse_lane_root_gather_f64(C.byref(d["root"]), _lib.ptr(factor), _lib.ptr(bufs["S"]), B, s), "root_gather")
                _lib.check(lib.thb_potrf_f64(_lib.ptr(bufs["S"]), None, None, _lib.ptr(bufs["info_root"]), B, d["nt"], _lib.ptr(bufs["ws"]),
                                             bufs["ws"].numel(), s), "root_potrf")
                torch.maximum(info, torch.where(bufs["info_root"] > 0, bufs["info_root"] + int(self._root[2]["root_start"]), bufs["info_root"]),
                              out=info)
        else:
            _lib.check(lib.thb_gram_f64(C.byref(d["gram"]), B, _lib.ptr(A_val), nnz, _lib.ptr(b), m, _lib.ptr(factor), P.data_size,
                                        _lib.ptr(Atb), None, s), "gram(sparse)")
            if alpha is not None:
                _lib.check(lib.thb_sparse_damp_f64(C.byref(d["plan"]), _lib.ptr(factor), _lib.ptr(alpha), _lib.ptr(beta), B, s), "sparse_damp")
            _lib.check(lib.thb_sparse_factor_f64(C.byref(d["plan"]), _lib.ptr(factor), _lib.ptr(diag), _lib.ptr(info), B, s), "sparse_factor")
        self._keep = (A_val, b, alpha, beta)
        return Atb

    def _substitute(self, rhs: torch.Tensor) -> torch.Tensor:
        d, P = self._dev, self._plan
        bufs = d["bufs"]
        B, layout = bufs["key"]
        if layout == "front":
            return self._substitute_front(rhs)
        lib = _lib.load()
        rhs = rhs.contiguous()
        x = torch.empty(B, P.n, dtype=torch.float64, device=rhs.device)
        pieces = C.byref(d["pieces"]) if (layout != "item" and "pieces" in d) else None
        if layout in ("lane", "lane_tiled") and pieces is not None:
            s = _lib.stream_ptr()
            lp, F, D, W = C.byref(d[layout]), _lib.ptr(bufs["factor"]), _lib.ptr(bufs["diag"]), _lib.ptr(bufs["work"])
            _lib.check(lib.thb_sparse_lane_piece_forward_f64(lp, pieces, F, D, _lib.ptr(rhs), W, B, s), "piece_forward")
            _lib.check(lib.thb_sparse_lane_piece_backward_f64(lp, pieces, F, D, W, _lib.ptr(x), B, s), "piece_backward")
        elif layout in ("lane", "lane_tiled"):
            _lib.check(lib.thb_sparse_lane_solve_f64(C.byref(d[layout]), _lib.ptr(bufs["factor"]), _lib.ptr(bufs["diag"]), _lib.ptr(rhs), _lib.ptr(x),
                                                     _lib.ptr(bufs["work"]), B, _lib.stream_ptr()), "lane_solve")
        elif layout in _ROOT_LAYOUTS:
            s = _lib.stream_ptr()
            lp, rt = C.byref(d[layout]), C.byref(d["root"])
            F, D, W = _lib.ptr(bufs["factor"]), _lib.ptr(bufs["diag"]), _lib.ptr(bufs["work"])
            if pieces is not None:
                _lib.check(lib.thb_sparse_lane_piece_forward_f64(lp, pieces, F, D, _lib.ptr(rhs), W, B, s), "piece_forward")
            else:
                _lib.check(lib.thb_sparse_lane_forward_f64(lp, F, D, _lib.ptr(rhs), W, B, s), "lane_forward")
            _lib.check(lib.thb_sparse_lane_root_rhs_f64(lp, rt, F, _lib.ptr(rhs), W, _lib.ptr(bufs["rhs_root"]), B, s), "root_rhs")
            _lib.check(lib.thb_potrs_f64(_lib.ptr(bufs["rhs_root"]), _lib.ptr(bufs["x_root"]), B, d["nt"], _lib.ptr(bufs["ws"]), bufs["ws"].numel(), s),
                       "root_potrs")
            _lib.check(lib.thb_sparse_lane_root_scatter_f64(lp, rt, _lib.ptr(bufs["x_root"]), W, _lib.ptr(x), B, s), "root_scatter")
            if pieces is not None:
                _lib.check(lib.thb_sparse_lane_piece_backward_f64(lp, pieces, F, D, W, _lib.ptr(x), B, s), "piece_backward")
            else:
                _lib.check(lib.thb_sparse_lane_backward_f64(lp, F, D, W, _lib.ptr(x), B, s), "lane_backward")
        else:
            _lib.check(lib.thb_sparse_solve_f64(C.byref(d["plan"]), _lib.ptr(bufs["factor"]), _lib.ptr(bufs["diag"]), _lib.ptr(rhs), _lib.ptr(x),
                                                _lib.ptr(bufs["work"]), B, _lib.stream_ptr()), "sparse_solve")
        return x


BlockSparseSolver = BaspachoSparseSolver
CholmodSparseSolver = BaspachoSparseSolver
LUCudaSparseSolver = BaspachoSparseSolver
```

Baseline: 4.749.

## Fuse forward substitution into multifrontal factor kernel for small fronts

The small-front factorization kernel now assembles each front's right-hand side, including child update contributions, into the shared-memory panel and runs the forward triangular elimination in place right after factoring. This removes the separate forward-solve launch sweep and the reread of the factor from global memory. The Python path calls a combined factor+forward entry point and then only the backward sweep. Front prefetch also becomes opt-in by default, and the change adds shared-memory and register pressure plus extra synchronisation inside the factor kernel.

```diff
diff --git a/include/thb200.h b/include/thb200.h
--- a/include/thb200.h
+++ b/include/thb200.h
@@ -285,6 +285,14 @@
                          int32_t* info, int64_t B, thb_stream_t stream);
 int thb_front_solve_f64(const thb_front_plan* p, const int64_t* launches, int64_t num_launches, const double* factor, const double* rhs,
                         double* x, double* work, double* varena, int64_t B, thb_stream_t stream);
+int thb_front_factor_forward_f64(const thb_front_plan* p, const int64_t* launches, int64_t num_launches, double* factor, const double* ata,
+                                 int64_t ata_stride, const double* alpha, const double* beta, double* arena, void* dense_ws,
+                                 int64_t dense_ws_bytes, int32_t* info, const double* rhs, double* work, double* varena, int64_t B,
+                                 thb_stream_t stream);
+int thb_front_forward_f64(const thb_front_plan* p, const int64_t* launches, int64_t num_launches, const double* factor, const double* rhs,
+                          double* work, double* varena, int64_t B, thb_stream_t stream);
+int thb_front_backward_f64(const thb_front_plan* p, const int64_t* launches, int64_t num_launches, const double* factor, double* x,
+                           double* work, int64_t B, thb_stream_t stream);
 int64_t thb_potrf_partial_workspace_bytes(int64_t B, int64_t np);
 int thb_potrf_partial_inplace_f64(double* F, int64_t bstride, int64_t np, int32_t nb_piv, int32_t w_real, int32_t n_real, int32_t info_base,
                                   int32_t* info, int64_t B, void* workspace, int64_t workspace_bytes, thb_stream_t stream);
diff --git a/theseus_b200/_lib.py b/theseus_b200/_lib.py
--- a/theseus_b200/_lib.py
+++ b/theseus_b200/_lib.py
@@ -135,6 +135,10 @@
     "thb_front_small_smem_bytes": (c_i64, [c_i32, c_i32, c_i32]),
     "thb_front_factor_f64": (c_i32, [_PF, c_vp, c_i64, c_vp, c_vp, c_i64, c_vp, c_vp, c_vp, c_vp, c_i64, c_vp, c_i64, c_vp]),
     "thb_front_solve_f64": (c_i32, [_PF, c_vp, c_i64, c_vp, c_vp, c_vp, c_vp, c_vp, c_i64, c_vp]),
+    "thb_front_factor_forward_f64": (c_i32, [_PF, c_vp, c_i64, c_vp, c_vp, c_i64, c_vp, c_vp, c_vp, c_vp, c_i64, c_vp, c_vp, c_vp, c_vp,
+                                             c_i64, c_vp]),
+    "thb_front_forward_f64": (c_i32, [_PF, c_vp, c_i64, c_vp, c_vp, c_vp, c_vp, c_i64, c_vp]),
+    "thb_front_backward_f64": (c_i32, [_PF, c_vp, c_i64, c_vp, c_vp, c_vp, c_i64, c_vp]),
     "thb_potrf_partial_workspace_bytes": (c_i64, [c_i64, c_i64]),
     "thb_potrf_partial_inplace_f64": (c_i32, [c_vp, c_i64, c_i64, c_i32, c_i32, c_i32, c_i32, c_vp, c_i64, c_vp, c_i64, c_vp]),
     "thb_solve_backward_f64": (c_i32, [c_i64, c_i64, c_i64, c_vp, c_vp, c_vp, c_vp, c_vp, c_vp, c_vp, c_i32, c_vp, c_vp, c_vp]),
diff --git a/theseus_b200/csrc/thb_front.cu b/theseus_b200/csrc/thb_front.cu
--- a/theseus_b200/csrc/thb_front.cu
+++ b/theseus_b200/csrc/thb_front.cu
@@ -60,6 +60,10 @@
   int prefetch;
   const double* ata;
   int64_t ata_stride;
+  const double* rhs;
+  double* work;
+  double* v_cur;
+  const double* v_child;
 };
 
 __device__ __forceinline__ double front_panel_in(const FrontArgs& a, const double* Lg, int64_t poff, int64_t item, int64_t e) {
@@ -171,8 +175,71 @@
 
 struct FrontChild {
   const double* src;
-  int ldg, lo, hi, pad;
+  int ldg, lo, hi, uoff;
 };
+
+__device__ __forceinline__ double front_warp_trsv_lower(const double* T, int ld, double ui, int cw, int lane) {
+  const double rd = lane < cw ? 1.0 / T[lane * ld + lane] : 0.0;
+  for (int k = 0; k < cw; k++) {
+    const double yk = __shfl_sync(0xffffffffu, ui * rd, k);
+    if (lane == k) ui = yk;
+    else if (lane > k && lane < cw) ui -= T[lane * ld + k] * yk;
+  }
+  return ui;
+}
+
+struct FrontRowsGlobal {
+  static constexpr bool kInPanel = false;
+  const double* L;
+  int w;
+  double* T;
+  __device__ __forceinline__ const double* row(int i) const { return L + (int64_t)i * w; }
+  __device__ __forceinline__ const double* diag(int k0, int cw, int tid, int nthreads, int* ld) const {
+    for (int e = tid; e < cw * cw; e += nthreads) {
+      const int i = e / cw, j = e - i * cw;
+      T[i * 33 + j] = L[(int64_t)(k0 + i) * w + k0 + j];
+    }
+    *ld = 33;
+    return T;
+  }
+};
+struct FrontRowsPanel {
+  static constexpr bool kInPanel = true;
+  const double* PN;
+  int ldp, w, shift;
+  __device__ __forceinline__ const double* row(int i) const { return PN + (i < w ? i : i + shift) * ldp; }
+  __device__ __forceinline__ const double* diag(int k0, int, int, int, int* ld) const {
+    *ld = ldp;
+    return PN + k0 * ldp + k0;
+  }
+};
+
+template <int THREADS, typename Rows>
+__device__ __forceinline__ void front_forward_elim(const Rows& R, double* u, int us, int w, int r, int tid, int lane) {
+  for (int k0 = 0; k0 < w; k0 += 32) {
+    const int cw = min(32, w - k0);
+    int ld;
+    const double* T = R.diag(k0, cw, tid, THREADS, &ld);
+    __syncthreads();
+    if (tid < 32) {
+      const double ui = front_warp_trsv_lower(T, ld, lane < cw ? u[(k0 + lane) * us] : 0.0, cw, lane);
+      if (lane < cw) u[(k0 + lane) * us] = ui;
+    }
+    __syncthreads();
+    for (int i = k0 + cw + tid; i < r; i += THREADS) {
+      const double* row = R.row(i) + k0;
+      double s = 0.0;
+      if constexpr (Rows::kInPanel) {
+#pragma unroll 2
+        for (int k = 0; k < cw; k++) s += row[k] * u[(k0 + k) * us];
+      } else {
+        for (int k = 0; k < cw; k++) s += row[k] * u[(k0 + k) * us];
+      }
+      u[i * us] -= s;
+    }
+    __syncthreads();
+  }
+}
 
 template <int THREADS>
 __global__ void __launch_bounds__(THREADS, 1024 / THREADS) front_small_kernel(FrontArgs a) {
@@ -191,7 +258,6 @@
   const int f_cb_ld = (int)FD[6];
   const int c_begin = (int)(FD[7] & 0xffffffffLL);
   const int nch = min((int)(FD[7] >> 32), FRONT_MAX_CHILDREN);
-  (void)t;
   const int b16 = (b + 15) & ~15, w8 = (w + 7) & ~7;
   const int ldp = front_pad_ld(w8);
   const int prow = w8 + b16 + 8;
@@ -208,6 +274,7 @@
       ch[q].ldg = cld;
       ch[q].lo = (int)PC[2];
       ch[q].hi = (int)PC[3];
+      ch[q].uoff = (int)PC[5];
     }
     const int32_t* inv = p.c_inv + PC[4];
     for (int l = tid; l < r; l += THREADS) INV[q * r + l] = inv[l];
@@ -216,6 +283,14 @@
   for (int e = tid; e < prow * ldp; e += THREADS) sm[e] = 0.0;
   THB_PDL_WAIT();
 #ifndef THB_SIMT_EMU
+  if (a.rhs != nullptr) {
+    for (int i = tid; i < w; i += THREADS) asm volatile("prefetch.global.L2 [%0];\n" ::"l"(a.rhs + item * p.n + p.perm[f_first + i]));
+    for (int q = 0; q < nch; q++) {
+      const int64_t* PC = p.pc + (int64_t)(c_begin + q) * 6;
+      const double* cu = a.v_child + item * p.varena_size + PC[5];
+      for (int off = tid * 16; off < (int)(PC[1] >> 32); off += THREADS * 16) asm volatile("prefetch.global.L2 [%0];\n" ::"l"(cu + off));
+    }
+  }
   for (int q = 0; a.prefetch != 0 && q < nch; q++) {
     const int64_t* PC = p.pc + (int64_t)(c_begin + q) * 6;
     const double* csrc = a.arena_child + item * p.arena_size + PC[0];
@@ -264,6 +339,19 @@
         if (ii[u] >= 0) PN[(ii[u] < w ? ii[u] : ii[u] + (w8 - w)) * ldp + jj[u]] = v[u];
     }
   }
+  double* U = PN + w8;
+  if (a.rhs != nullptr) {
+    for (int i = tid; i < r; i += THREADS) {
+      double v = i < w ? a.rhs[item * p.n + p.perm[f_first + i]] : 0.0;
+      for (int q = 0; q < nch; q++) {
+        if (i >= ch[q].lo && i <= ch[q].hi) {
+          const int k = INV[q * r + i];
+          if (k >= 0) v += a.v_child[item * p.varena_size + ch[q].uoff + k];
+        }
+      }
+      U[i * ldp] = v;
+    }
+  }
   __syncthreads();
   const int nbk = w8 / 8, nrt = (w8 + b16) / 8;
   for (int jb = 0; jb < nbk; jb++) {
@@ -281,6 +369,12 @@
       i += di; j += dj;
       if (j >= w) { j -= w; i++; }
     }
+  }
+  if (a.rhs != nullptr) {
+    front_forward_elim<THREADS>(FrontRowsPanel{PN, ldp, w, w8 - w}, U, ldp, w, r, tid, lane);
+    for (int i = tid; i < w; i += THREADS) a.work[item * p.n + f_first + i] = U[i * ldp];
+    double* ub = a.v_cur + item * p.varena_size + p.f_u_off[t];
+    for (int i = tid; i < b; i += THREADS) ub[i] = U[(w + i) * ldp];
   }
   if (b == 0) return;
   double* dst = a.arena_cur + item * p.arena_size + f_cb_off;
@@ -508,15 +602,6 @@
   int stage_doubles;
 };
 
-__device__ __forceinline__ double front_warp_trsv_lower(const double* T, double ui, int cw, int lane) {
-  const double rd = lane < cw ? 1.0 / T[lane * 33 + lane] : 0.0;
-  for (int k = 0; k < cw; k++) {
-    const double yk = __shfl_sync(0xffffffffu, ui * rd, k);
-    if (lane == k) ui = yk;
-    else if (lane > k && lane < cw) ui -= T[lane * 33 + k] * yk;
-  }
-  return ui;
-}
 __device__ __forceinline__ double front_warp_trsv_upper(const double* T, double ti, int cw, int lane) {
   const double rd = lane < cw ? 1.0 / T[lane * 33 + lane] : 0.0;
   for (int k = cw - 1; k >= 0; k--) {
@@ -531,7 +616,7 @@
 __global__ void __launch_bounds__(THREADS) front_forward_kernel(FrontSolveArgs a) {
   extern __shared__ double sm[];
   const thb_front_plan& p = a.p;
-  const int tid = threadIdx.x, lane = tid & 31, warp = tid >> 5;
+  const int tid = threadIdx.x, lane = tid & 31;
   const int64_t item = blockIdx.x;
   THB_PDL_TRIGGER();
   const int64_t* FD = p.fd + (int64_t)(a.s0 + blockIdx.y) * 8;
@@ -561,26 +646,7 @@
     }
   }
   __syncthreads();
-  for (int k0 = 0; k0 < w; k0 += 32) {
-    const int cw = min(32, w - k0);
-    for (int e = tid; e < cw * cw; e += THREADS) {
-      const int i = e / cw, j = e - i * cw;
-      T[i * 33 + j] = Lg[(int64_t)(k0 + i) * w + k0 + j];
-    }
-    __syncthreads();
-    if (warp == 0) {
-      const double ui = front_warp_trsv_lower(T, lane < cw ? u[k0 + lane] : 0.0, cw, lane);
-      if (lane < cw) u[k0 + lane] = ui;
-    }
-    __syncthreads();
-    for (int i = k0 + cw + tid; i < r; i += THREADS) {
-      const double* row = Lg + (int64_t)i * w + k0;
-      double s = 0.0;
-      for (int k = 0; k < cw; k++) s += row[k] * u[k0 + k];
-      u[i] -= s;
-    }
-    __syncthreads();
-  }
+  front_forward_elim<THREADS>(FrontRowsGlobal{Lg, w, T}, u, 1, w, r, tid, lane);
   for (int i = tid; i < w; i += THREADS) a.work[item * p.n + first + i] = u[i];
   if (b > 0) {
     double* ub = a.v_cur + item * p.varena_size + p.f_u_off[t];
@@ -667,15 +733,44 @@
   return 0;
 }
 
-}
-
-extern "C" {
-
-int64_t thb_front_small_smem_bytes(int32_t w, int32_t b, int32_t nchildren) { return thb::front_smem_doubles(w, b, nchildren) * 8; }
-
-int thb_front_factor_f64(const thb_front_plan* p, const int64_t* launches, int64_t num_launches, double* factor, const double* ata,
-                         int64_t ata_stride, const double* alpha, const double* beta, double* arena, void* dense_ws, int64_t dense_ws_bytes,
-                         int32_t* info, int64_t B, thb_stream_t stream) {
+static int front_solve_launch(const thb_front_plan* p, const int64_t* L, int pass, const double* factor, const double* rhs, double* x,
+                              double* work, double* varena, int64_t B, cudaStream_t cs) {
+  static size_t fw_set[3] = {0, 0, 0}, bw_set[3] = {0, 0, 0};
+  static const int64_t stage_cap = [] { const char* e = getenv("THB_SOLVE_STAGE"); return e != nullptr ? (int64_t)atoll(e) : (int64_t)0; }();
+  const int depth = (int)L[0], cls = (int)L[1], begin = (int)L[2], count = (int)L[3];
+  FrontSolveArgs a;
+  a.p = *p; a.s0 = begin; a.B = B; a.factor = factor; a.rhs = rhs; a.x = x; a.work = work;
+  a.v_cur = varena != nullptr ? varena + (int64_t)(depth & 1) * B * p->varena_size : nullptr;
+  a.v_child = varena != nullptr ? varena + (int64_t)((depth + 1) & 1) * B * p->varena_size : nullptr;
+  const int kc = cls > 2 ? 2 : cls;
+  const int threads = front_threads_of_class(kc);
+  const int64_t r_max = L[5];
+  const int64_t stage = (cls < 3 && L[6] > 0) ? (L[6] < stage_cap ? L[6] : stage_cap) : 0;
+  a.stage_doubles = (int)stage;
+  const size_t smem = (size_t)(((r_max + 1) & ~1LL) + 32 * 33 + 1 + threads + 2 + stage + 2) * 8;
+  const dim3 grid((unsigned)B, (unsigned)count);
+  if (pass == 0) {
+    if (kc == 0) { int rc = front_set_smem(front_forward_kernel<64>, smem, &fw_set[0]); if (rc) return rc;
+                   FRONT_LAUNCH(front_forward_kernel<64>, grid, 64, smem, cs, a); }
+    else if (kc == 1) { int rc = front_set_smem(front_forward_kernel<128>, smem, &fw_set[1]); if (rc) return rc;
+                        FRONT_LAUNCH(front_forward_kernel<128>, grid, 128, smem, cs, a); }
+    else { int rc = front_set_smem(front_forward_kernel<256>, smem, &fw_set[2]); if (rc) return rc;
+           FRONT_LAUNCH(front_forward_kernel<256>, grid, 256, smem, cs, a); }
+  } else {
+    if (kc == 0) { int rc = front_set_smem(front_backward_kernel<64>, smem, &bw_set[0]); if (rc) return rc;
+                   FRONT_LAUNCH(front_backward_kernel<64>, grid, 64, smem, cs, a); }
+    else if (kc == 1) { int rc = front_set_smem(front_backward_kernel<128>, smem, &bw_set[1]); if (rc) return rc;
+                        FRONT_LAUNCH(front_backward_kernel<128>, grid, 128, smem, cs, a); }
+    else { int rc = front_set_smem(front_backward_kernel<256>, smem, &bw_set[2]); if (rc) return rc;
+           FRONT_LAUNCH(front_backward_kernel<256>, grid, 256, smem, cs, a); }
+  }
+  THB_CHECK_LAUNCH();
+  return THB_OK;
+}
+
+static int front_factor(const thb_front_plan* p, const int64_t* launches, int64_t num_launches, double* factor, const double* ata,
+                        int64_t ata_stride, const double* alpha, const double* beta, double* arena, void* dense_ws, int64_t dense_ws_bytes,
+                        int32_t* info, const double* rhs, double* work, double* varena, int64_t B, thb_stream_t stream) {
   if (p == nullptr || launches == nullptr || factor == nullptr || arena == nullptr || info == nullptr || B < 0) return THB_ERR_BAD_ARG;
   if (B == 0 || p->S == 0) return THB_OK;
   if (B > 65535LL * 32768LL) return THB_ERR_UNSUPPORTED;
@@ -687,17 +782,21 @@
   static int front_prefetch_flag = -1;
   if (front_prefetch_flag < 0) {
     const char* e = getenv("THB_FRONT_PREFETCH");
-    front_prefetch_flag = (e != nullptr && e[0] == '0') ? 0 : 1;
-  }
+    front_prefetch_flag = (e != nullptr && e[0] == '1') ? 1 : 0;
+  }
+  static const int fuse_max = [] { const char* e = getenv("THB_FRONT_FUSE_MAX"); return e != nullptr ? atoi(e) : 1024; }();
   for (int64_t l = 0; l < num_launches; l++) {
     const int64_t* L = launches + l * THB_FRONT_LAUNCH_COLS;
     const int depth = (int)L[0], cls = (int)L[1], begin = (int)L[2], count = (int)L[3];
-    thb::FrontArgs a;
+    FrontArgs a;
     a.p = *p; a.s0 = begin; a.B = B; a.factor = factor; a.alpha = alpha; a.beta = beta; a.info = info;
     a.ata = (ata != nullptr && p->pmap != nullptr) ? ata : nullptr; a.ata_stride = ata_stride;
     a.prefetch = front_prefetch_flag;
     a.arena_cur = arena + (int64_t)(depth & 1) * B * p->arena_size;
     a.arena_child = arena + (int64_t)((depth + 1) & 1) * B * p->arena_size;
+    a.rhs = rhs; a.work = work;
+    a.v_cur = rhs != nullptr ? varena + (int64_t)(depth & 1) * B * p->varena_size : nullptr;
+    a.v_child = rhs != nullptr ? varena + (int64_t)((depth + 1) & 1) * B * p->varena_size : nullptr;
     if (cls < 3) {
       const size_t smem = (size_t)L[4];
 #ifndef THB_SIMT_EMU
@@ -705,23 +804,32 @@
 #endif
       const dim3 grid((unsigned)B, (unsigned)count);
       if (count > 65535) return THB_ERR_UNSUPPORTED;
-      if (cls == 0 && thr_cls[0] == 64) {
-        int rc = thb::front_set_smem(thb::front_small_kernel<64>, smem, &smem_set[0]); if (rc) return rc;
-        FRONT_LAUNCH(thb::front_small_kernel<64>, grid, 64, smem, cs, a);
-      } else if ((cls == 0 && thr_cls[0] == 128) || (cls == 1 && thr_cls[1] == 128)) {
-        int rc = thb::front_set_smem(thb::front_small_kernel<128>, smem, &smem_set[1]); if (rc) return rc;
-        FRONT_LAUNCH(thb::front_small_kernel<128>, grid, 128, smem, cs, a);
-      } else if (cls <= 1 || smem <= 56 * 1024) {
-        int rc = thb::front_set_smem(thb::front_small_kernel<256>, smem, &smem_set[2]); if (rc) return rc;
-        FRONT_LAUNCH(thb::front_small_kernel<256>, grid, 256, smem, cs, a);
-      } else if (smem <= 113 * 1024) {
-        int rc = thb::front_set_smem(thb::front_small_kernel<512>, smem, &smem_set[3]); if (rc) return rc;
-        FRONT_LAUNCH(thb::front_small_kernel<512>, grid, 512, smem, cs, a);
+      const int threads = (cls == 0 && thr_cls[0] == 64) ? 64
+                          : ((cls == 0 && thr_cls[0] == 128) || (cls == 1 && thr_cls[1] == 128)) ? 128
+                          : (cls <= 1 || smem <= 56 * 1024) ? 256 : (smem <= 113 * 1024 ? 512 : 1024);
+      const bool fused = rhs != nullptr && threads <= fuse_max;
+      if (!fused) a.rhs = nullptr;
+      if (threads == 64) {
+        int rc = front_set_smem(front_small_kernel<64>, smem, &smem_set[0]); if (rc) return rc;
+        FRONT_LAUNCH(front_small_kernel<64>, grid, 64, smem, cs, a);
+      } else if (threads == 128) {
+        int rc = front_set_smem(front_small_kernel<128>, smem, &smem_set[1]); if (rc) return rc;
+        FRONT_LAUNCH(front_small_kernel<128>, grid, 128, smem, cs, a);
+      } else if (threads == 256) {
+        int rc = front_set_smem(front_small_kernel<256>, smem, &smem_set[2]); if (rc) return rc;
+        FRONT_LAUNCH(front_small_kernel<256>, grid, 256, smem, cs, a);
+      } else if (threads == 512) {
+        int rc = front_set_smem(front_small_kernel<512>, smem, &smem_set[3]); if (rc) return rc;
+        FRONT_LAUNCH(front_small_kernel<512>, grid, 512, smem, cs, a);
       } else {
-        int rc = thb::front_set_smem(thb::front_small_kernel<1024>, smem, &smem_set[4]); if (rc) return rc;
-        FRONT_LAUNCH(thb::front_small_kernel<1024>, grid, 1024, smem, cs, a);
+        int rc = front_set_smem(front_small_kernel<1024>, smem, &smem_set[4]); if (rc) return rc;
+        FRONT_LAUNCH(front_small_kernel<1024>, grid, 1024, smem, cs, a);
       }
       THB_CHECK_LAUNCH();
+      if (rhs != nullptr && !fused) {
+        const int rc = front_solve_launch(p, L, 0, factor, rhs, nullptr, work, varena, B, cs);
+        if (rc != THB_OK) return rc;
+      }
     } else {
       const int64_t np = L[5], nb_piv = L[6], fr_off = L[7], first = L[8];
       const int t = (int)L[9];
@@ -730,19 +838,45 @@
       return THB_ERR_UNSUPPORTED;
 #else
       if (dense_ws == nullptr || np % 128 != 0 || np > 8192) return THB_ERR_BAD_ARG;
-      const size_t smem = (size_t)thb::ASM_ROWS * np * 8;
-      int rc = thb::front_set_smem(thb::front_assemble_kernel, smem, &asm_set); if (rc) return rc;
-      thb::front_assemble_kernel<<<dim3((unsigned)B, (unsigned)(np / thb::ASM_ROWS)), thb::ASM_THREADS, smem, cs>>>(a, t);
+      const size_t smem = (size_t)ASM_ROWS * np * 8;
+      int rc = front_set_smem(front_assemble_kernel, smem, &asm_set); if (rc) return rc;
+      front_assemble_kernel<<<dim3((unsigned)B, (unsigned)(np / ASM_ROWS)), ASM_THREADS, smem, cs>>>(a, t);
       THB_CHECK_LAUNCH();
       rc = thb_potrf_partial_inplace_f64(a.arena_cur + fr_off, p->arena_size, np, (int32_t)nb_piv, (int32_t)L[10], (int32_t)(nb_piv * 64 + L[11]),
                                          (int32_t)first, info, B, dense_ws, dense_ws_bytes, stream);
       if (rc != THB_OK) return rc;
-      thb::front_extract_kernel<<<dim3((unsigned)B, 8), 256, 0, cs>>>(a, t);
+      front_extract_kernel<<<dim3((unsigned)B, 8), 256, 0, cs>>>(a, t);
       THB_CHECK_LAUNCH();
+      if (rhs != nullptr) {
+        rc = front_solve_launch(p, L, 0, factor, rhs, nullptr, work, varena, B, cs);
+        if (rc != THB_OK) return rc;
+      }
 #endif
     }
   }
   return THB_OK;
+}
+
+}
+
+extern "C" {
+
+int64_t thb_front_small_smem_bytes(int32_t w, int32_t b, int32_t nchildren) { return thb::front_smem_doubles(w, b, nchildren) * 8; }
+
+int thb_front_factor_f64(const thb_front_plan* p, const int64_t* launches, int64_t num_launches, double* factor, const double* ata,
+                         int64_t ata_stride, const double* alpha, const double* beta, double* arena, void* dense_ws, int64_t dense_ws_bytes,
+                         int32_t* info, int64_t B, thb_stream_t stream) {
+  return thb::front_factor(p, launches, num_launches, factor, ata, ata_stride, alpha, beta, arena, dense_ws, dense_ws_bytes, info, nullptr,
+                           nullptr, nullptr, B, stream);
+}
+
+int thb_front_factor_forward_f64(const thb_front_plan* p, const int64_t* launches, int64_t num_launches, double* factor, const double* ata,
+                                 int64_t ata_stride, const double* alpha, const double* beta, double* arena, void* dense_ws,
+                                 int64_t dense_ws_bytes, int32_t* info, const double* rhs, double* work, double* varena, int64_t B,
+                                 thb_stream_t stream) {
+  if (rhs == nullptr || work == nullptr || varena == nullptr) return THB_ERR_BAD_ARG;
+  return thb::front_factor(p, launches, num_launches, factor, ata, ata_stride, alpha, beta, arena, dense_ws, dense_ws_bytes, info, rhs, work,
+                           varena, B, stream);
 }
 
 int thb_front_solve_f64(const thb_front_plan* p, const int64_t* launches, int64_t num_launches, const double* factor, const double* rhs,
@@ -751,44 +885,34 @@
       B < 0)
     return THB_ERR_BAD_ARG;
   if (B == 0 || p->S == 0) return THB_OK;
+  const int rc = thb_front_forward_f64(p, launches, num_launches, factor, rhs, work, varena, B, stream);
+  if (rc != THB_OK) return rc;
+  return thb_front_backward_f64(p, launches, num_launches, factor, x, work, B, stream);
+}
+
+int thb_front_forward_f64(const thb_front_plan* p, const int64_t* launches, int64_t num_launches, const double* factor, const double* rhs,
+                          double* work, double* varena, int64_t B, thb_stream_t stream) {
+  if (p == nullptr || launches == nullptr || factor == nullptr || rhs == nullptr || work == nullptr || varena == nullptr || B < 0)
+    return THB_ERR_BAD_ARG;
+  if (B == 0 || p->S == 0) return THB_OK;
   cudaStream_t cs = thb_cs(stream);
-  static size_t fw_set[3] = {0, 0, 0}, bw_set[3] = {0, 0, 0};
-  static const int64_t stage_cap = [] { const char* e = getenv("THB_SOLVE_STAGE"); return e != nullptr ? (int64_t)atoll(e) : (int64_t)0; }();
-  for (int pass = 0; pass < 2; pass++) {
-    for (int64_t q = 0; q < num_launches; q++) {
-      const int64_t l = pass == 0 ? q : num_launches - 1 - q;
-      const int64_t* L = launches + l * THB_FRONT_LAUNCH_COLS;
-      const int depth = (int)L[0], cls = (int)L[1], begin = (int)L[2], count = (int)L[3];
-      thb::FrontSolveArgs a;
-      a.p = *p; a.s0 = begin; a.B = B; a.factor = factor; a.rhs = rhs; a.x = x; a.work = work;
-      a.v_cur = varena + (int64_t)(depth & 1) * B * p->varena_size;
-      a.v_child = varena + (int64_t)((depth + 1) & 1) * B * p->varena_size;
-      const int kc = cls > 2 ? 2 : cls;
-      const int threads = thb::front_threads_of_class(kc);
-      const int64_t r_max = L[5];
-      const int64_t stage = (cls < 3 && L[6] > 0) ? (L[6] < stage_cap ? L[6] : stage_cap) : 0;
-      a.stage_doubles = (int)stage;
-      const size_t smem = (size_t)(((r_max + 1) & ~1LL) + 32 * 33 + 1 + threads + 2 + stage + 2) * 8;
-      const dim3 grid((unsigned)B, (unsigned)count);
-      if (pass == 0) {
-        if (kc == 0) { int rc = thb::front_set_smem(thb::front_forward_kernel<64>, smem, &fw_set[0]); if (rc) return rc;
-                       FRONT_LAUNCH(thb::front_forward_kernel<64>, grid, 64, smem, cs, a); }
-        else if (kc == 1) { int rc = thb::front_set_smem(thb::front_forward_kernel<128>, smem, &fw_set[1]); if (rc) return rc;
-                            FRONT_LAUNCH(thb::front_forward_kernel<128>, grid, 128, smem, cs, a); }
-        else { int rc = thb::front_set_smem(thb::front_forward_kernel<256>, smem, &fw_set[2]); if (rc) return rc;
-               FRONT_LAUNCH(thb::front_forward_kernel<256>, grid, 256, smem, cs, a); }
-      } else {
-        if (kc == 0) { int rc = thb::front_set_smem(thb::front_backward_kernel<64>, smem, &bw_set[0]); if (rc) return rc;
-                       FRONT_LAUNCH(thb::front_backward_kernel<64>, grid, 64, smem, cs, a); }
-        else if (kc == 1) { int rc = thb::front_set_smem(thb::front_backward_kernel<128>, smem, &bw_set[1]); if (rc) return rc;
-                            FRONT_LAUNCH(thb::front_backward_kernel<128>, grid, 128, smem, cs, a); }
-        else { int rc = thb::front_set_smem(thb::front_backward_kernel<256>, smem, &bw_set[2]); if (rc) return rc;
-               FRONT_LAUNCH(thb::front_backward_kernel<256>, grid, 256, smem, cs, a); }
-      }
-      THB_CHECK_LAUNCH();
-    }
+  for (int64_t q = 0; q < num_launches; q++) {
+    const int rc = thb::front_solve_launch(p, launches + q * THB_FRONT_LAUNCH_COLS, 0, factor, rhs, nullptr, work, varena, B, cs);
+    if (rc != THB_OK) return rc;
   }
   return THB_OK;
 }
 
-}
+int thb_front_backward_f64(const thb_front_plan* p, const int64_t* launches, int64_t num_launches, const double* factor, double* x,
+                           double* work, int64_t B, thb_stream_t stream) {
+  if (p == nullptr || launches == nullptr || factor == nullptr || x == nullptr || work == nullptr || B < 0) return THB_ERR_BAD_ARG;
+  if (B == 0 || p->S == 0) return THB_OK;
+  cudaStream_t cs = thb_cs(stream);
+  for (int64_t q = num_launches - 1; q >= 0; q--) {
+    const int rc = thb::front_solve_launch(p, launches + q * THB_FRONT_LAUNCH_COLS, 1, factor, nullptr, x, work, nullptr, B, cs);
+    if (rc != THB_OK) return rc;
+  }
+  return THB_OK;
+}
+
+}
diff --git a/theseus_b200/sparse_solver.py b/theseus_b200/sparse_solver.py
--- a/theseus_b200/sparse_solver.py
+++ b/theseus_b200/sparse_solver.py
@@ -181,7 +181,7 @@
                          max_np=int(big[:, 5].max()) if len(big) else 0)
         return self._dev
 
-    def _numeric_front(self, A_val, b, alpha, beta):
+    def _numeric_front(self, A_val, b, alpha, beta, forward=False):
         B, device = A_val.shape[0], A_val.device
         d = self._device_plan(device)
         P = self._plan
@@ -212,11 +212,15 @@
         L = d["launches"]
         for c0 in range(0, B, chunk):
             nb = min(chunk, B - c0)
-            _lib.check(lib.thb_front_factor_f64(
-                C.byref(d["front"]), L.ctypes.data, L.shape[0], _lib.ptr(factor[c0:]), _lib.ptr(ata[c0:]), self._ata_size,
-                _lib.ptr(alpha[c0:]) if alpha is not None else None,
-                _lib.ptr(beta[c0:]) if beta is not None else None, _lib.ptr(bufs["arena"]), _lib.ptr(bufs["ws"]) if d["max_np"] else None,
-                bufs["ws"].numel(), _lib.ptr(info[c0:]), nb, s), "front_factor")
+            args = (C.byref(d["front"]), L.ctypes.data, L.shape[0], _lib.ptr(factor[c0:]), _lib.ptr(ata[c0:]), self._ata_size,
+                    _lib.ptr(alpha[c0:]) if alpha is not None else None,
+                    _lib.ptr(beta[c0:]) if beta is not None else None, _lib.ptr(bufs["arena"]), _lib.ptr(bufs["ws"]) if d["max_np"] else None,
+                    bufs["ws"].numel(), _lib.ptr(info[c0:]))
+            if forward:
+                _lib.check(lib.thb_front_factor_forward_f64(*args, _lib.ptr(Atb[c0:]), _lib.ptr(bufs["work"][c0:]), _lib.ptr(bufs["varena"]), nb, s),
+                           "front_factor_forward")
+            else:
+                _lib.check(lib.thb_front_factor_f64(*args, nb, s), "front_factor")
         self._keep = (A_val, b, alpha, beta)
         return Atb
 
@@ -233,6 +237,19 @@
             _lib.check(lib.thb_front_solve_f64(C.byref(d["front"]), L.ctypes.data, L.shape[0], _lib.ptr(bufs["factor"][c0:]), _lib.ptr(rhs[c0:]),
                                                _lib.ptr(x[c0:]), _lib.ptr(bufs["work"][c0:]), _lib.ptr(bufs["varena"]), nb, _lib.stream_ptr()),
                        "front_solve")
+        return x
+
+    def _backward_front(self):
+        d, P = self._dev, self._plan
+        bufs = d["bufs"]
+        B, chunk = bufs["key"][0], bufs["chunk"]
+        lib = _lib.load()
+        x = torch.empty(B, P.n, dtype=torch.float64, device=bufs["work"].device)
+        L = d["launches"]
+        for c0 in range(0, B, chunk):
+            nb = min(chunk, B - c0)
+            _lib.check(lib.thb_front_backward_f64(C.byref(d["front"]), L.ctypes.data, L.shape[0], _lib.ptr(bufs["factor"][c0:]), _lib.ptr(x[c0:]),
+                                                  _lib.ptr(bufs["work"][c0:]), nb, _lib.stream_ptr()), "front_backward")
         return x
 
     def _lane_struct(self, ln, dev, device):
@@ -280,8 +297,12 @@
         alpha = beta = None
         if damping is not None:
             alpha, beta = convert_to_alpha_beta_damping_tensors(damping, damping_eps, ellipsoidal_damping, A64.shape[0], A64.device, torch.float64)
-        Atb = self._numeric(A64, b64, alpha, beta)
-        x = self._substitute(Atb)
+        if self.layout_for(A64.shape[0]) == "front":
+            self._numeric_front(A64, b64, alpha, beta, forward=True)
+            x = self._backward_front()
+        else:
+            Atb = self._numeric(A64, b64, alpha, beta)
+            x = self._substitute(Atb)
         self._last_info = self._dev["bufs"]["info"]
         if not getattr(self, "defer_info_check", False):
             self.check_info()
```

Measured after the change: 5.063, median of 6. 6.6% higher.
